# peterrum/deal-and-ceed-on-gpu

Hardware: AMD Instinct MI355X
Metric: BP5 DoFs/sec per CG iter (p=4, ~1e8 DoFs) + % HBM roofline at 1/2/4/8 GPUs (higher is better)
Workload: dtype f64

## Files before the change

deal-and-ceed-on-gpu_amd/csrc/bp5_device.hip:

```cpp
#include "bp5_device.hpp"


extern "C" int bp5_device_count(int *count)
{
  if (!count) return fail(BP5_ERR_INVALID, "null argument");
  int c = 0;
  hipError_t e = hipGetDeviceCount(&c);
  if (e != hipSuccess) { *count = 0; return fail(BP5_ERR_NO_DEVICE, hipGetErrorString(e)); }
  *count = c;
  return BP5_OK;
}
extern "C" int bp5_vec_alloc(size_t n, double **out)
{
  if (!out) return fail(BP5_ERR_INVALID, "null argument");
  HIP_TRY(hipMalloc((void **)out, std::max<size_t>(n, 1) * sizeof(double)));
  HIP_TRY(hipMemset(*out, 0, std::max<size_t>(n, 1) * sizeof(double)));
  HIP_TRY(hipStreamSynchronize(nullptr));
  return BP5_OK;
}
extern "C" int bp5_vec_free(double *v) { HIP_TRY(hipFree(v)); return BP5_OK; }
extern "C" int bp5_copy_h2d(void *dst, const void *src, size_t bytes) { HIP_TRY(hipMemcpy(dst, src, bytes, hipMemcpyHostToDevice)); return BP5_OK; }
extern "C" int bp5_copy_d2h(void *dst, const void *src, size_t bytes) { HIP_TRY(hipMemcpy(dst, src, bytes, hipMemcpyDeviceToHost)); return BP5_OK; }

static void tuning_from_environment(bp5_mf *mf);
// ... 701 lines not shown
    uint32_t *ra = lat.data() + g * BLOCK_LATTICE_WORDS, *rb = ra + BLOCK_LATTICE_WORDS;
    ra[55] = f.len << 16 | f.s_out;
    rb[56] = f.len << 16 | f.s_in;
    dp.h_carry_dof[g] = f.dof; dp.h_carry_len[g] = f.len;
    ++n_faces;
  }
  if (!n_faces) { dp.h_carry_dof.clear(); dp.h_carry_len.clear(); }
  return n_faces;
}

int build_carry_tables(bp5_mf *mf, bp5_mf::DevPlan *dp, const std::vector<uint32_t> &wb, uint32_t n_wg, bool two_parts, bp5_mf::DevPlan::CombineTables *out)
{
  std::vector<std::pair<uint32_t, uint32_t>> cut;
  for (int part = 0; part < (two_parts ? 2 : 1); ++part) {
    const uint32_t *w = wb.data() + (size_t)part * (n_wg + 1);
    for (uint32_t i = 0; i < n_wg; ++i)
      for (uint32_t g = w[i]; g + 1 < w[i + 1]; ++g)
        if (dp->h_carry_len[g]) cut.emplace_back(dp->h_carry_dof[g], dp->h_carry_len[g]);
  }
  std::sort(cut.begin(), cut.end());
  const std::vector<uint32_t> &st = dp->h_cr_start, &d0 = dp->h_cr_dof0, &so = dp->h_cr_soff, &sl = dp->h_cr_slots;
  const size_t nr = d0.size();
  std::vector<uint32_t> start, dof0, soff, slots;
  uint32_t ord = 0, owned = 0;
  size_t ci = 0;
  auto emit = [&](size_t r, uint32_t first, uint32_t count) {
    if (!count) return;
    const uint32_t base = d0[r] & 0x7fffffffu;
    start.push_back(ord);
    dof0.push_back(first | (d0[r] & 0x80000000u));
    soff.push_back((uint32_t)slots.size());
    for (uint32_t q = so[r]; q < so[r + 1]; ++q) slots.push_back(sl[q] + (first - base));
    ord += count;
    if (first < mf->n_owned) owned += std::min(count, mf->n_owned - first);
  };
  for (size_t r = 0; r < nr; ++r) {
    uint32_t first = d0[r] & 0x7fffffffu;
    const uint32_t end = first + (st[r + 1] - st[r]);
    while (ci < cut.size() && cut[ci].first + cut[ci].second <= first) ++ci;
    size_t c = ci;
    while (c < cut.size() && cut[c].first < end) {
      const uint32_t c0 = std::max(cut[c].first, first), c1 = std::min(cut[c].first + cut[c].second, end);
      emit(r, first, c0 - first);
      first = c1;
      ++c;
    }
    emit(r, first, end - first);
  }
  start.push_back(ord);
  soff.push_back((uint32_t)slots.size());
  BP5_TRY(upload_combine_tables(start, dof0, soff, slots, out));
  out->n_shared_owned = owned;
  return BP5_OK;
}

int get_plan_raw(bp5_mf *mf, int key, bp5_mf::DevPlan **dpo, int default_block)
{
  auto it = mf->plans.find(key);
  if (it == mf->plans.end()) {
    TeamPlanHost h;
    if (key < 0 && mf->n_local() >= (1ull << 30)) return fail(BP5_ERR_UNSUPPORTED, "block plan needs fewer than 2^30 local DoFs");
    if (key > 0) BP5_TRY(build_team_plan(mf->h_l2g.data(), mf->n_cells, mf->n3, mf->n_local(), key, h));
    else if (!mf->h_block_off.empty())
      BP5_TRY(build_team_plan(mf->h_l2g.data(), mf->n_cells, mf->n3, mf->n_local(), 0, h, mf->h_block_off.data(),
                              (uint32_t)mf->h_block_off.size() - 1, -key));
    else BP5_TRY(build_team_plan(mf->h_l2g.data(), mf->n_cells, mf->n3, mf->n_local(), default_block, h, nullptr, 0, -key));
    bp5_mf::DevPlan dp;
    BP5_TRY(upload(&dp.off, h.off.data(), h.off.size()));
    BP5_TRY(upload(&dp.dofs, h.dofs.data(), h.dofs.size()));
    std::vector<uint32_t> run_off, runs;
    if (key < 0) {
      std::vector<uint32_t> lat;
      std::vector<uint16_t> cpos;
      const bool lattice_enabled = mf->tune[BP5_TUNE_LATTICE_INDICES] != 0;
      dp.n_lattice_blocks = detect_lattice_blocks(mf->h_l2g.data(), mf->degree + 1, h.group_cell_off, h.off, h.dofs, lat, cpos);
      std::vector<CarryFace> faces;
      if (dp.n_lattice_blocks && dp.n_lattice_blocks == (uint32_t)(h.off.size() - 1)) faces = find_carry_faces(mf, mf->degree, h, lat);
      auto face_edge = [&](size_t g, uint32_t slot) {
        if (faces.empty()) return false;
        if (faces[g].len && (slot == faces[g].s_out || slot == faces[g].s_out + faces[g].len)) return true;
        return g > 0 && faces[g - 1].len && (slot == faces[g - 1].s_in || slot == faces[g - 1].s_in + faces[g - 1].len);
      };
      run_off.assign(h.off.size(), 0);
      for (size_t g = 0; g + 1 < h.off.size(); ++g) {
        uint32_t start = h.off[g];
        for (uint32_t i = h.off[g]; i < h.off[g + 1]; ++i) {
          const bool con = mf->h_constrained[h.dofs[i] & 0x7fffffffu];
          if (i == h.off[g] || h.dofs[i] != h.dofs[i - 1] + 1 || i - start == (1u << BLOCK_PACK_OFF_BITS) ||
              con != (bool)mf->h_constrained[h.dofs[i - 1] & 0x7fffffffu] || face_edge(g, i - h.off[g])) {
            start = i;
            runs.push_back(i - h.off[g]);
            runs.push_back(h.dofs[i] | (con ? BLOCK_DOF_CONSTRAINED : 0u));
          }
        }
        run_off[g + 1] = (uint32_t)(runs.size() / 2);
        dp.max_runs = std::max(dp.max_runs, run_off[g + 1] - run_off[g]);
      }
      const int n = mf->degree + 1, n2 = n * n;
      auto off = [&](int k, int ab) { return k < 2 * (n / 2) ? (k / 2) * (2 * n2) + 2 * ab + (k & 1) : (n / 2) * (2 * n2) + ab; };
      std::vector<uint16_t> pos2(h.pos.size()), packed(dp.max_runs <= (uint32_t)BLOCK_PACK_MAX_RUNS ? h.pos.size() : 0);
      std::vector<uint32_t> gidx(h.pos.size());
#pragma omp parallel
      {
        std::vector<uint16_t> run_of_slot;
#pragma omp for schedule(dynamic, 16)
        for (int64_t g = 0; g < (int64_t)h.group_cell_off.size() - 1; ++g) {
          const uint32_t nr = run_off[g + 1] - run_off[g], m = h.off[g + 1] - h.off[g];
          if (!packed.empty()) {
            run_of_slot.assign(m, 0);
            for (uint32_t r = 0; r < nr; ++r) {
              const uint32_t s0 = runs[2 * (run_off[g] + r)], s1 = r + 1 < nr ? runs[2 * (run_off[g] + r + 1)] : m;
              for (uint32_t sl = s0; sl < s1; ++sl) run_of_slot[sl] = (uint16_t)r;
            }
          }
          for (size_t c = h.group_cell_off[g]; c < h.group_cell_off[g + 1]; ++c)
            for (int k = 0; k < n; ++k)
              for (int ab = 0; ab < n2; ++ab) {
                const size_t from = c * mf->n3 + (size_t)k * n2 + ab, to = c * mf->n3 + off(k, ab);
                pos2[to] = h.pos[from];
                gidx[to] = mf->h_l2g[from];
                if (!packed.empty()) {
                  const uint32_t sl = h.pos[from], r = run_of_slot[sl];
                  packed[to] = (uint16_t)(r << BLOCK_PACK_OFF_BITS | (sl - runs[2 * (run_off[g] + r)]));
                }
              }
        }
      }
      BP5_TRY(upload(&dp.pos, pos2.data(), pos2.size()));
      BP5_TRY(upload(&dp.gidx, gidx.data(), gidx.size()));
      if (!packed.empty()) BP5_TRY(upload(&dp.packed, packed.data(), packed.size()));
      if (!packed.empty() && dp.n_lattice_blocks && lattice_enabled) {
        if (!faces.empty()) mark_carry_faces(h, faces, run_off, runs, lat, dp);
        BP5_TRY(upload(&dp.lattice, lat.data(), lat.size()));
        BP5_TRY(upload(&dp.cell_pos, cpos.data(), cpos.size()));
      } else
        dp.n_lattice_blocks = 0;
    } else
      BP5_TRY(upload(&dp.pos, h.pos.data(), h.pos.size()));
    BP5_TRY(upload(&dp.cell_round, h.cell_round.data(), h.cell_round.size()));
    BP5_TRY(upload(&dp.team_rounds, h.team_rounds.data(), h.team_rounds.size()));
    BP5_TRY(upload(&dp.sh_dof, h.sh_dof.data(), h.sh_dof.size()));
    BP5_TRY(upload(&dp.sh_off, h.sh_off.data(), h.sh_off.size()));
    BP5_TRY(upload(&dp.sh_slot, h.sh_slot.data(), h.sh_slot.size()));
    HIP_TRY(hipMalloc((void **)&dp.partial, std::max<size_t>(h.dofs.size(), 1) * sizeof(double)));
    HIP_TRY(hipMemsetAsync(dp.partial, 0, std::max<size_t>(h.dofs.size(), 1) * sizeof(double), mf->stream));
    BP5_TRY(upload(&dp.cell_off, h.group_cell_off.data(), h.group_cell_off.size()));
    if (key < 0) {
      BP5_TRY(upload(&dp.pass_cell, h.pass_cell.data(), h.pass_cell.size()));
      BP5_TRY(upload(&dp.pass_off, h.pass_off.data(), h.pass_off.size()));
      dp.h_cost.assign(h.pass_off.size(), 0.0);
      for (size_t g = 0; g + 1 < h.pass_off.size(); ++g) {
        const double passes = h.pass_off[g + 1] - h.pass_off[g], rounds = h.team_rounds[g], m = h.off[g + 1] - h.off[g];
        dp.h_cost[g + 1] = dp.h_cost[g] + passes * (1.0 + 0.18 * (rounds - 1.0)) + 1.5 * m / 4913.0 + 1.0;
      }
      runs.push_back(0); runs.push_back(0);
      BP5_TRY(upload(&dp.run_off, run_off.data(), run_off.size()));
      BP5_TRY(upload(&dp.runs, runs.data(), runs.size()));
    }
    dp.n_shared = (uint32_t)h.sh_dof.size();
    dp.n_shared_owned = (uint32_t)(std::lower_bound(h.sh_dof.begin(), h.sh_dof.end(), mf->n_owned) - h.sh_dof.begin());
    if (dp.n_shared) {
      std::vector<uint32_t> start, dof0, soff, slots, tile;
      const size_t ns = h.sh_dof.size();
      for (size_t i = 0; i < ns; ++i) {
        const uint32_t b = h.sh_off[i], e = h.sh_off[i + 1];
        bool cont = i > 0 && h.sh_dof[i] == h.sh_dof[i - 1] + 1 && (e - b) == (h.sh_off[i] - h.sh_off[i - 1]) &&
                    mf->h_constrained[h.sh_dof[i]] == mf->h_constrained[h.sh_dof[i - 1]];
        for (uint32_t q = 0; cont && q < e - b; ++q) cont = h.sh_slot[b + q] == h.sh_slot[h.sh_off[i - 1] + q] + 1;
        if (!cont) {
          start.push_back((uint32_t)i);
          dof0.push_back(h.sh_dof[i] | (mf->h_constrained[h.sh_dof[i]] ? 0x80000000u : 0u));
          soff.push_back((uint32_t)slots.size());
          slots.insert(slots.end(), h.sh_slot.begin() + b, h.sh_slot.begin() + e);
        }
      }
      start.push_back((uint32_t)ns);
      soff.push_back((uint32_t)slots.size());
      bp5_mf::DevPlan::CombineTables ct;
      BP5_TRY(upload_combine_tables(start, dof0, soff, slots, &ct));
      dp.cr_start = ct.start; dp.cr_dof0 = ct.dof0; dp.cr_soff = ct.soff; dp.cr_slots = ct.slots; dp.cr_tile = ct.tile;
      if (!dp.h_carry_len.empty()) { dp.h_cr_start = start; dp.h_cr_dof0 = dof0; dp.h_cr_soff = soff; dp.h_cr_slots = slots; }
    }
    dp.covers_all = h.covers_all;
    dp.n_groups = (uint32_t)h.group_cell_off.size() - 1;
    for (uint32_t g = 0; g < dp.n_groups; ++g) dp.max_list = std::max(dp.max_list, h.off[g + 1] - h.off[g]);
    it = mf->plans.emplace(key, dp).first;
  }
// ... 518 lines not shown
  for (hipEvent_t &e : mf->ev_halo) HIP_TRY(hipEventCreateWithFlags(&e, hipEventDisableTiming));
  int can = 0;
  if (hipDeviceGetAttribute(&can, hipDeviceAttributeCanUseStreamWaitValue, mf->device) != hipSuccess) can = 0;
  if (can && !mf->d_signal) {
    HIP_TRY(hipMalloc((void **)&mf->d_signal, 4 * sizeof(unsigned long long)));
    HIP_TRY(hipMemset(mf->d_signal, 0, 4 * sizeof(unsigned long long)));
    HIP_TRY(hipStreamSynchronize(nullptr));
    mf->signal_target = 0;
  }
  if (can) {
    mf->signal_target += 1;
    hipLaunchKernelGGL(wait_value_probe_producer, dim3(1), dim3(64), 0, mf->stream, mf->d_signal, mf->d_signal + 1, mf->d_signal + 2, 200000LL );
    KERNEL_CHECK();
    const bool waited = hipStreamWaitValue64(mf->comm_stream, mf->d_signal, mf->signal_target, hipStreamWaitValueGte, ~0ull) == hipSuccess;
    if (waited) { hipLaunchKernelGGL(wait_value_probe_consumer, dim3(1), dim3(64), 0, mf->comm_stream, mf->d_signal + 1); KERNEL_CHECK(); }
    else (void)hipGetLastError();
    HIP_TRY(hipStreamSynchronize(mf->stream));
    HIP_TRY(hipStreamSynchronize(mf->comm_stream));
    unsigned long long released_mid_kernel = 0;
    HIP_TRY(hipMemcpy(&released_mid_kernel, mf->d_signal + 2, sizeof(released_mid_kernel), hipMemcpyDeviceToHost));
    if (!waited || !released_mid_kernel) can = 0;
  }
  mf->wait_value_ok = can;
  mf->can_wait_value = can && mf->tune[BP5_TUNE_BOUNDARY_FIRST] != 0;
  return BP5_OK;
}
extern "C" int bp5_mf_wait_value_available(bp5_mf *mf, int *available)
{
  if (!mf || !available) return fail(BP5_ERR_INVALID, "null argument");
  HIP_TRY(hipSetDevice(mf->device));
  BP5_TRY(halo_streams(mf));
  *available = mf->wait_value_ok == 1;
  return BP5_OK;
}
static int env_int(const char *name, int fallback)
{
  const char *e = getenv(name);
  return (e && *e) ? atoi(e) : fallback;
}
static void tuning_from_environment(bp5_mf *mf)
{
  mf->tune[BP5_TUNE_LATTICE_INDICES] = env_int("BP5_LATTICE_INDICES", 1) != 0;
  mf->tune[BP5_TUNE_EARLY_GATHER] = env_int("BP5_EARLY_GATHER", 1) != 0;
  mf->tune[BP5_TUNE_COMBINE_SIGNAL] = env_int("BP5_COMBINE_SIGNAL", 0) == 1;
  { const char *e = getenv("BP5_BOUNDARY_FIRST"); mf->tune[BP5_TUNE_BOUNDARY_FIRST] = !(e && !strcmp(e, "launches")); }
  mf->tune[BP5_TUNE_FOLD_SMALL] = env_int("BP5_FOLD_SMALL", 1) != 0;
  { const int u = env_int("BP5_UPDATE_UNROLL", 1); mf->tune[BP5_TUNE_UPDATE_UNROLL] = (u == 2 || u == 4) ? u : 1; }
  mf->tune[BP5_TUNE_UPDATE_FLAT] = env_int("BP5_UPDATE_FLAT", 1) != 0;
  { const int v = env_int("BP5_UPDATE_NT", -1); mf->tune[BP5_TUNE_UPDATE_NT] = v < 0 ? -1 : v != 0; }
  { const int v = env_int("BP5_COMBINE_WG_PER_CU", 16); mf->tune[BP5_TUNE_COMBINE_WG_PER_CU] = (v >= 0 && v <= 32) ? v : 16; }
  mf->tune[BP5_TUNE_INTERIOR_STORES] = env_int("BP5_INTERIOR_STORES", 1) != 0;
  mf->tune[BP5_TUNE_GHOST_COMBINE_ON_COMM] = env_int("BP5_GHOST_COMBINE_ON_COMM", 0) != 0;
  mf->tune[BP5_TUNE_FACE_CARRY] = env_int("BP5_FACE_CARRY", 1) != 0;
}
extern "C" int bp5_mf_set_tuning(bp5_mf *mf, int knob, int value)
{
  if (!mf || knob < 0 || knob >= BP5_TUNE_COUNT) return fail(BP5_ERR_INVALID, "unknown tuning knob");
  switch (knob) {
    case BP5_TUNE_UPDATE_UNROLL:
      if (value != 1 && value != 2 && value != 4) return fail(BP5_ERR_INVALID, "BP5_TUNE_UPDATE_UNROLL: 1, 2 or 4");
      break;
    case BP5_TUNE_UPDATE_NT:
      if (value < -1 || value > 1) return fail(BP5_ERR_INVALID, "BP5_TUNE_UPDATE_NT: -1, 0 or 1");
      break;
    case BP5_TUNE_COMBINE_WG_PER_CU:
      if (value < 0 || value > 32) return fail(BP5_ERR_INVALID, "BP5_TUNE_COMBINE_WG_PER_CU: 0 ... 32");
      break;
    case BP5_TUNE_LATTICE_INDICES:
      if (value != 0 && value != 1) return fail(BP5_ERR_INVALID, "switch: 0 or 1");
      if (value != mf->tune[knob] && mf->plans.count(-block_cpt(mf))) return fail(BP5_ERR_INVALID, "BP5_TUNE_LATTICE_INDICES: the block plan of this handle is already built");
      break;
    default:
      if (value != 0 && value != 1) return fail(BP5_ERR_INVALID, "switch: 0 or 1");
  }
  mf->tune[knob] = value;
  if (knob == BP5_TUNE_BOUNDARY_FIRST && mf->wait_value_ok >= 0) mf->can_wait_value = mf->wait_value_ok == 1 && value != 0;
  return BP5_OK;
}
extern "C" int bp5_mf_get_tuning(const bp5_mf *mf, int knob, int *value)
{
  if (!mf || !value || knob < 0 || knob >= BP5_TUNE_COUNT) return fail(BP5_ERR_INVALID, "unknown tuning knob");
  *value = mf->tune[knob];
  return BP5_OK;
}
extern "C" int bp5_mf_set_overlap(bp5_mf *mf, int mode)
{
  if (!mf || mode < 0 || mode > 2) return fail(BP5_ERR_INVALID, "bad argument");
  mf->overlap = mode;
  return BP5_OK;
}
static bool overlap_wanted(const bp5_mf *mf) { return mf->overlap == 1 || (mf->overlap == 2 && mf->n_interior >= 1000000u); }
static int gather_exchange(bp5_mf *mf, double *v, bool on_comm_stream);
static int gather_start(bp5_mf *mf, double *v, bool on_comm_stream)
{
  HIP_TRY(hipSetDevice(mf->device));
  BP5_TRY(halo_streams(mf));
  const uint32_t ns = mf->send_off.back();
  if (ns) {
    hipLaunchKernelGGL(pack_kernel, dim3((ns + 255) / 256), dim3(256), 0, mf->stream, mf->d_send_idx, ns, v, mf->d_sendbuf);
    KERNEL_CHECK();
  }
  return gather_exchange(mf, v, on_comm_stream);
}
extern "C" int bp5_halo_gather_start(bp5_mf *mf, double *v)
{
  if (!mf || !v) return fail(BP5_ERR_INVALID, "null argument");
  if (mf->neighbors.empty()) return BP5_OK;
  if (!mf->comm) return fail(BP5_ERR_INVALID, "halo exchange needs bp5_mf_set_comm");
  return gather_start(mf, v, overlap_wanted(mf));
}
static int gather_exchange(bp5_mf *mf, double *v, bool on_comm_stream)
{
  mf->overlap_now = on_comm_stream;
  hipStream_t cs = mf->overlap_now ? mf->comm_stream : mf->stream;
  if (mf->overlap_now) {
    HIP_TRY(hipEventRecord(mf->ev_halo[0], mf->stream));
// ... 368 lines not shown
extern "C" int bp5_event_elapsed_ms(bp5_event *a, bp5_event *b, double *ms)
{
  if (!a || !b || !ms) return fail(BP5_ERR_INVALID, "null argument");
  HIP_TRY(hipEventSynchronize(b->ev));
  float f = 0.f;
  HIP_TRY(hipEventElapsedTime(&f, a->ev, b->ev));
  *ms = f;
  return BP5_OK;
}
extern "C" int bp5_event_destroy(bp5_event *e)
{
  if (!e) return BP5_OK;
  hipEventDestroy(e->ev);
  delete e;
  return BP5_OK;
}

static int ensure_ws(bp5_mf *mf)
{
  if (mf->ws_g) return BP5_OK;
  const size_t stagger = 0;
  const size_t nb = (std::max<size_t>(mf->n_local(), 2) * sizeof(double) + 4095) / 4096 * 4096;
  char *base = nullptr;
  HIP_TRY(hipMalloc((void **)&base, 3 * nb + 2 * stagger + 4096));
  HIP_TRY(hipMemsetAsync(base, 0, 3 * nb + 2 * stagger + 4096, mf->stream));
  mf->ws_base = base;
  mf->ws_g = (double *)base;
  mf->ws_d = (double *)(base + nb + stagger);
  mf->ws_h = (double *)(base + 2 * nb + 2 * stagger);
  return BP5_OK;
}

struct ApplyProfile {
  bp5_mf *mf;
  bool on;
  int used = 0;
  static constexpr int MAX_PROFILED = 512;
  int mark(int k)
  {
    if (!on) return BP5_OK;
    if (used >= 4 * MAX_PROFILED) { on = false; return BP5_OK; }
    while ((size_t)used + 4 > mf->ev_pool.size()) { hipEvent_t e; HIP_TRY(hipEventCreate(&e)); mf->ev_pool.push_back(e); }
    HIP_TRY(hipEventRecord(mf->ev_pool[used + k], mf->stream));
    return BP5_OK;
  }
};

struct SolveState {
  ApplyProfile prof;
  int exchange = EXCHANGE_NONE;
  bool two_parts = false;
  bool gather_in_flight = false;
  bool dst_prezeroed = false, copies_dirichlet = false;
  bool phase_on = false;
  int phase_it = 0;
  uint8_t phase_recorded[bp5_mf::PhaseProfile::MAX_ITERS] = {};
};

static int phase_mark(bp5_mf *mf, SolveState &ss, int k)
{
  if (!ss.phase_on || ss.phase_it >= bp5_mf::PhaseProfile::MAX_ITERS) return BP5_OK;
  HIP_TRY(hipEventRecord(mf->phase.ev[(size_t)ss.phase_it * bp5_mf::PhaseProfile::MARKS + k], mf->stream));
  ss.phase_recorded[ss.phase_it] |= (uint8_t)(1u << k);
  return BP5_OK;
}

static int fused_unsplit(bp5_mf *mf, SolveState &ss, ApplyCall &call, const double *coef, const double *src, double *dst)
{
  ApplyProfile &prof = ss.prof;
  if (prof.on) call.mark_event = mf->ev_pool[prof.used + 2];
  BP5_TRY(launch_apply(mf, call, coef, src, dst));
  if (!call.mark_recorded) BP5_TRY(prof.mark(2));
  BP5_TRY(prof.mark(3));
  if (prof.on) prof.used += 4;
  BP5_TRY(phase_mark(mf, ss, 3));
  BP5_TRY(halo_streams(mf));
  BP5_TRY(scatter_exchange(mf, dst, false));
  return scatter_add_finish(mf, dst, call.fuse);
}
static int fused_ghost_rows_first(bp5_mf *mf, SolveState &ss, ApplyCall &call, const double *coef, const double *src, double *dst)
{
  ApplyProfile &prof = ss.prof;
  bp5_mf::DevPlan *dp = nullptr;
  BP5_TRY(get_plan_raw(mf, -block_cpt(mf), &dp));
  BP5_TRY(halo_streams(mf));
  call.combine_later = true;
  BP5_TRY(launch_apply(mf, call, coef, src, dst));
  BP5_TRY(prof.mark(2));
  const bool combine_signal = mf->tune[BP5_TUNE_COMBINE_SIGNAL] != 0;
  const bool one_combine = combine_signal && mf->can_wait_value == 1 && mf->n_ghost && mf->d_signal && dp->n_shared > dp->n_shared_owned && dp->cr_tile && !call.csr_combine;
  if (one_combine) {
    BP5_TRY(launch_combine(mf, call, dp, dst, true, COMBINE_GHOST_THEN_OWNED));
    HIP_TRY(hipStreamWaitValue64(mf->comm_stream, mf->d_signal, mf->signal_target, hipStreamWaitValueGte, ~0ull));
    BP5_TRY(scatter_exchange(mf, dst, true, true));
  } else if (mf->tune[BP5_TUNE_GHOST_COMBINE_ON_COMM] && mf->n_ghost) {
    HIP_TRY(hipEventRecord(mf->ev_halo[2], mf->stream));
    HIP_TRY(hipStreamWaitEvent(mf->comm_stream, mf->ev_halo[2], 0));
    BP5_TRY(launch_combine(mf, call, dp, dst, true, COMBINE_GHOST, true));
    BP5_TRY(scatter_exchange(mf, dst, true, true));
    BP5_TRY(launch_combine(mf, call, dp, dst, true, COMBINE_OWNED));
  } else {
    if (mf->n_ghost) BP5_TRY(launch_combine(mf, call, dp, dst, true, COMBINE_GHOST));
    BP5_TRY(scatter_exchange(mf, dst, true));
    BP5_TRY(launch_combine(mf, call, dp, dst, true, mf->n_ghost ? COMBINE_OWNED : COMBINE_ALL));
  }
  BP5_TRY(prof.mark(3));
// ... 41 lines not shown
  if (ss.gather_in_flight) { ss.gather_in_flight = false; BP5_TRY(bp5_halo_gather_finish(mf, src)); }
  else {
    BP5_TRY(gather_start(mf, src, false));
    BP5_TRY(bp5_halo_gather_finish(mf, src));
  }
  BP5_TRY(phase_mark(mf, ss, 2));
  BP5_TRY(ss.prof.mark(0));
  BP5_TRY(ss.prof.mark(1));
  FuseState fuse;
  fuse.p = src; fuse.r = fuse_r;
  ApplyCall call;
  call.c0 = 0; call.c1 = mf->n_cells; call.overwrite = true;
  call.fuse = &fuse;
  call.exchange = ss.exchange;
  call.two_parts = ss.two_parts;
  if (ss.exchange == EXCHANGE_BOUNDARY_FIRST) BP5_TRY(fused_boundary_first(mf, ss, call, coef, src, dst));
  else if (ss.exchange == EXCHANGE_GHOST_ROWS_FIRST) BP5_TRY(fused_ghost_rows_first(mf, ss, call, coef, src, dst));
  else BP5_TRY(fused_unsplit(mf, ss, call, coef, src, dst));
  *n_cols = fuse.n_cols;
  if (!fuse.ghosts_zeroed) BP5_TRY(bp5_halo_zero_ghosts(mf, src));
  return BP5_OK;
}

static int solver_vmult(bp5_mf *mf, SolveState &ss, const double *coef, double *src, double *dst, bool zero, const double *fuse_r = nullptr,
                        uint32_t *n_cols = nullptr)
{
  ApplyProfile &prof = ss.prof;
  const bool dist = mf->has_neighbors();
  const bool fusing = n_cols != nullptr;
  if (dist && fusing) return fused_vmult_distributed(mf, ss, coef, src, dst, fuse_r, n_cols);
  ApplyCall call;
  call.c0 = 0; call.c1 = mf->n_cells;
  if (dist) {
    BP5_TRY(prof.mark(0));
    BP5_TRY(prof.mark(1));
    if (prof.on) call.mark_event = mf->ev_pool[prof.used + 2];
    BP5_TRY(apply_overlapped(mf, call, coef, src, dst, zero));
    if (!call.mark_recorded) BP5_TRY(prof.mark(2));
    BP5_TRY(prof.mark(3));
    if (prof.on) prof.used += 4;
    BP5_TRY(bp5_halo_zero_ghosts(mf, src));
    return bp5_copy_constrained(mf, src, dst);
  }
  const bool owner_scatter = variant_overwrites(mf, effective_variant(mf, 0, mf->n_cells));
  BP5_TRY(prof.mark(0));
  if (zero && !owner_scatter) {
    if (!ss.dst_prezeroed) HIP_TRY(hipMemsetAsync(dst, 0, mf->n_local() * sizeof(double), mf->stream));
    zero = false;
    call.dst_known_zero = true;
  }
  BP5_TRY(prof.mark(1));
  if (prof.on) call.mark_event = mf->ev_pool[prof.used + 2];
  FuseState fuse;
  if (fusing) { fuse.p = src; fuse.r = fuse_r; call.fuse = &fuse; }
  call.overwrite = zero;
  BP5_TRY(launch_apply(mf, call, coef, src, dst));
  if (fusing) *n_cols = fuse.n_cols;
  if (!call.mark_recorded) BP5_TRY(prof.mark(2));
  BP5_TRY(prof.mark(3));
  if (prof.on) prof.used += 4;
  if (fusing) return BP5_OK;
  if (ss.copies_dirichlet) return BP5_OK;
  return bp5_copy_constrained(mf, src, dst);
}

static int poll_state(bp5_mf *mf)
{
  HIP_TRY(hipMemcpyAsync(mf->h_st, mf->d_st, ST_COUNT * sizeof(int), hipMemcpyDeviceToHost, mf->stream));
  HIP_TRY(hipMemcpyAsync(mf->h_sc, mf->d_sc, SC_COUNT * sizeof(double), hipMemcpyDeviceToHost, mf->stream));
  HIP_TRY(hipStreamSynchronize(mf->stream));
  return BP5_OK;
}

static int solve_begin(bp5_mf *mf, const bp5_cg_params *prm, const ApplyProfile &prof)
{
  hipStream_t s = mf->stream;
  if (prof.on) {
    const size_t want = 4 * (size_t)std::min(prm->max_iter, ApplyProfile::MAX_PROFILED);
    while (mf->ev_pool.size() < want) { hipEvent_t e; HIP_TRY(hipEventCreate(&e)); mf->ev_pool.push_back(e); }
  }
  mf->h_sc[SC_TOL] = prm->abs_tol;
  HIP_TRY(hipMemcpyAsync(mf->d_sc + SC_TOL, mf->h_sc + SC_TOL, sizeof(double), hipMemcpyHostToDevice, s));
  mf->h_st[ST_MAXIT] = prm->max_iter;
  HIP_TRY(hipMemcpyAsync(mf->d_st + ST_MAXIT, mf->h_st + ST_MAXIT, sizeof(int), hipMemcpyHostToDevice, s));
  HIP_TRY(hipStreamSynchronize(s));
  HIP_TRY(hipEventRecord(mf->ev_solve[0], s));
  return BP5_OK;
}
static int solve_finish(bp5_mf *mf, const ApplyProfile &prof, bool fused_dots, int exchange_schedule, bool own_operator, bp5_cg_result *res)
{
  HIP_TRY(hipEventRecord(mf->ev_solve[1], mf->stream));
  BP5_TRY(poll_state(mf));
  float ms = 0.f;
  HIP_TRY(hipEventElapsedTime(&ms, mf->ev_solve[0], mf->ev_solve[1]));
  memset(res, 0, sizeof(*res));
  res->iterations = mf->h_st[ST_ITER];
  res->residual = mf->h_sc[SC_RES];
  res->initial_residual = mf->h_sc[SC_RES0];
  res->solve_ms = ms;
  res->apply_launches = prof.used / 4;
  res->dot_products_fused = fused_dots ? 1 : 0;
  res->exchange_schedule = exchange_schedule;
  if (prof.on && prof.used) {
    double tot = 0.0, tot_op = 0.0;
    for (int k = 0; k < prof.used; k += 4) {
      float t = 0.f;
      HIP_TRY(hipEventElapsedTime(&t, mf->ev_pool[k + 1], mf->ev_pool[k + 2]));
      tot += t;
      HIP_TRY(hipEventElapsedTime(&t, mf->ev_pool[k], mf->ev_pool[k + 3]));
      tot_op += t;
    }
    res->apply_ms_avg = tot / (prof.used / 4);
    res->operator_ms_avg = tot_op / (prof.used / 4);
  }
  if (own_operator) strncpy(res->apply_kernel, mf->last_apply_kernel, sizeof(res->apply_kernel) - 1);
  if (mf->h_st[ST_BREAKDOWN]) return fail(BP5_ERR_BREAKDOWN, "CG breakdown: p.Ap is zero or NaN");
  return BP5_OK;
}

static int user_vmult(ApplyProfile &prof, bp5_vmult_fn user, void *user_ctx, double *src, double *dst)
{
  BP5_TRY(prof.mark(0));
  BP5_TRY(prof.mark(1));
  const int st = user(user_ctx, dst, src);
  if (st != BP5_OK) return fail(st, "the operator's vmult callback reported a failure");
  BP5_TRY(prof.mark(2));
  BP5_TRY(prof.mark(3));
  if (prof.on) prof.used += 4;
  return BP5_OK;
}

struct OperatorPlan {
  bool dist = false;
  bool fused_dots = false;
  bool fold_small = false;
  bool prezero = false;
  int schedule = 0;
};
static int plan_operator(bp5_mf *mf, bool own_operator, bool fusable, SolveState &ss, OperatorPlan &op)
{
  op.dist = mf->has_neighbors();
  bool split = false, split_possible = false, late = false;
  if (own_operator && mf->cg_fusion && !mf->f32_metric()  && fusable && mf->geometry_mode == BP5_GEOM_MERGED6 &&
      is_default_block(mf, effective_variant(mf, 0, mf->n_cells))) {
    bp5_mf::DevPlan *dp = nullptr;
    BP5_TRY(get_plan_raw(mf, -block_cpt(mf), &dp));
    op.fused_dots = dp->packed && dp->covers_all && (dp->n_shared == 0 || dp->cr_tile);
    if (op.fused_dots && op.dist) {
      uint32_t b0_, b1_;
      split_possible = !mf->h_block_off.empty() && (mf->n_interior == 0 || mf->n_interior == mf->n_cells || block_aligned(mf, 0, mf->n_interior, &b0_, &b1_));
      split = split_possible && mf->overlap == 1;
      if (mf->overlap == 1 && !split) op.fused_dots = false;
      late = op.fused_dots && mf->overlap == 2 && (dp->n_shared == 0 || dp->cr_tile);
    }
  }
  ss.exchange = split ? EXCHANGE_BOUNDARY_FIRST : late ? EXCHANGE_GHOST_ROWS_FIRST : EXCHANGE_NONE;
  ss.two_parts = op.fused_dots && op.dist && split_possible;
  const bool fold_enabled = mf->tune[BP5_TUNE_FOLD_SMALL] != 0;
  op.fold_small = fold_enabled && !op.fused_dots && own_operator && !op.dist;
  op.prezero = op.fold_small && mf->n_ghost == 0 && !variant_overwrites(mf, effective_variant(mf, 0, mf->n_cells));
  ss.dst_prezeroed = op.prezero;
  ss.copies_dirichlet = op.fold_small;
  op.schedule = !op.dist ? 0 : split ? 2 : late ? 4 : op.fused_dots ? 1 : overlap_wanted(mf) ? 3 : 1;
  return BP5_OK;
}

struct PlainCG {
  int n_components = 1;
  size_t ld = 0;
  double *g = nullptr, *d = nullptr, *h = nullptr;
  const double *coef = nullptr;
  bp5_vmult_fn user = nullptr;
  void *user_ctx = nullptr;
  bool block = false, exchange = false;
  const double *diag = nullptr;
  bp5_vmult_fn precond = nullptr;
  void *precond_ctx = nullptr;
  double *z = nullptr;
  bool allreduce = true;
  double *history = nullptr;
  int history_cap = 0;
};
static int cg_solve_plain(bp5_mf *mf, const PlainCG &cg, const double *b, double *x, const bp5_cg_params *prm, bp5_cg_result *res)
{
  hipStream_t s = mf->stream;
  const size_t n = mf->n_owned, ld = cg.ld;
  const int nc = cg.n_components;
  double *g = cg.g, *d = cg.d, *h = cg.h, *z = cg.z;
  const double *diag = cg.diag;
  const int cols = PARTIAL_STRIDE / nc;
  const dim3 grid1(std::min(stream_grid(n, 1), cols), nc), grid2(std::min(stream_grid(n, 2), cols), nc), block(VB);
  const dim3 gridd = cg.block ? grid2 : dim3(stream_grid_flat(mf, n, 2));
  const int nblk1 = (int)grid1.x * nc, nblk2 = (int)grid2.x * nc;
  const int *no_flag = nullptr;
  SolveState ss{ApplyProfile{mf, prm->profile != 0 && !cg.precond}};
  ApplyProfile &prof = ss.prof;
  BP5_TRY(solve_begin(mf, prm, prof));
  OperatorPlan op;
  if (!cg.block && !cg.precond) BP5_TRY(plan_operator(mf, !cg.user, true, ss, op));
  else op.schedule = cg.user || !mf->has_neighbors() ? 0 : overlap_wanted(mf) ? 3 : 1;
  auto apply_A = [&](uint32_t *n_cols) -> int {
    if (cg.user) return user_vmult(prof, cg.user, cg.user_ctx, d, h);
    if (!cg.block) return solver_vmult(mf, ss, cg.coef, d, h, true, nullptr, op.fused_dots ? n_cols : nullptr);
    BP5_TRY(prof.mark(0));
    BP5_TRY(components_zero(mf, nc, ld, h));
    BP5_TRY(prof.mark(1));
    if (cg.exchange) BP5_TRY(components_apply_exchanged(mf, cg.coef, nc, ld, d, h, false));
// ... 53 lines not shown
    } else {
      hipLaunchKernelGGL(cg_update_kernel<true>, grid2, block, 0, s, x, g, d, h, diag, n, ld, mf->d_sc, mf->d_st, mf->d_partials, op.prezero);
      hipLaunchKernelGGL(finalize_kernel<2>, dim3(2), block, 0, s, mf->d_partials, nblk2, mf->d_sc + SC_GG, mf->d_st);
    }
    if (cg.allreduce) { KERNEL_CHECK(); BP5_TRY(bp5_comm_allreduce_sum(mf, mf->d_sc + SC_GG, 2)); }
    hipLaunchKernelGGL(cg_control_kernel, dim3(1), dim3(1), 0, s, mf->d_sc, mf->d_st);
    if (cg.history) hipLaunchKernelGGL(cg_record_kernel, dim3(1), dim3(1), 0, s, mf->d_sc, mf->d_st, cg.history, cg.history_cap);
    if (cg.precond) hipLaunchKernelGGL((cg_direction_kernel<true, false>), gridd, block, 0, s, d, z, diag, n, ld, mf->d_sc, mf->d_st);
    else hipLaunchKernelGGL((cg_direction_kernel<false, false>), gridd, block, 0, s, d, g, diag, n, ld, mf->d_sc, mf->d_st);
    KERNEL_CHECK();
    if (check > 0 && it % check == 0 && it < prm->max_iter) {
      BP5_TRY(poll_state(mf));
      if (mf->h_st[ST_DONE]) break;
    } else if (lagged_look && it < prm->max_iter) {
      const int slot = it % (DONE_LAG + 1);
      HIP_TRY(hipMemcpyAsync(mf->h_done + slot, mf->d_st + ST_DONE, sizeof(int), hipMemcpyDeviceToHost, s));
      HIP_TRY(hipEventRecord(mf->ev_done[slot], s));
      if (it > DONE_LAG) {
        const int seen = (it - DONE_LAG) % (DONE_LAG + 1);
        HIP_TRY(hipEventSynchronize(mf->ev_done[seen]));
        if (mf->h_done[seen]) break;
      }
    }
  }
  return solve_finish(mf, prof, op.fused_dots, op.schedule, !cg.user, res);
}

static int cg_solve_merged(bp5_mf *mf, const double *coef, bp5_vmult_fn user, void *user_ctx, const double *diag, const double *b, double *x,
                           const bp5_cg_params *prm, bp5_cg_result *res)
{
  const size_t n = mf->n_owned;
  const int grid2 = stream_grid(n, 2), grid1 = stream_grid(n, 1);
  hipStream_t s = mf->stream;
  double *g = mf->ws_g, *d = mf->ws_d, *h = mf->ws_h;
  SolveState ss{ApplyProfile{mf, prm->profile != 0}};
  ss.phase_on = prm->profile == 2;
  if (ss.phase_on) {
    const size_t want = (size_t)bp5_mf::PhaseProfile::MAX_ITERS * bp5_mf::PhaseProfile::MARKS;
    while (mf->phase.ev.size() < want) { hipEvent_t e; HIP_TRY(hipEventCreate(&e)); mf->phase.ev.push_back(e); }
  }
  BP5_TRY(solve_begin(mf, prm, ss.prof));
  OperatorPlan op;
  BP5_TRY(plan_operator(mf, !user, !diag, ss, op));
  const bool fused = op.fused_dots, dist_solve = op.dist, fold_small = op.fold_small, prezero = op.prezero;
  auto vmult = [&](double *src, double *dst, const double *fuse_r, uint32_t *n_cols) -> int {
    if (!user) return solver_vmult(mf, ss, coef, src, dst, true, fuse_r, n_cols);
    return user_vmult(ss.prof, user, user_ctx, src, dst);
  };
  const int check = prm->check_every;
  hipLaunchKernelGGL(cgm_init_kernel, dim3(grid1), dim3(VB), 0, s, b, x, g, d, h, diag, n, mf->d_partials, !(fused && !dist_solve));
  hipLaunchKernelGGL(finalize_kernel<2>, dim3(2), dim3(VB), 0, s, mf->d_partials, grid1, mf->d_sc + SC_GG, (const int *)nullptr);
  KERNEL_CHECK();
  BP5_TRY(bp5_comm_allreduce_sum(mf, mf->d_sc + SC_GG, 2));
  hipLaunchKernelGGL(cgm_init_control_kernel, dim3(1), dim3(1), 0, s, mf->d_sc, mf->d_st);
  KERNEL_CHECK();
  const int unroll = mf->tune[BP5_TUNE_UPDATE_UNROLL];
  const int gridu = stream_grid_flat(mf, n, 2 * unroll);
  const bool streaming = mf->tune[BP5_TUNE_UPDATE_NT] != 0;
  auto launch_update = [&](int mode) {
#define BP5_UPD(M, U, ZV, NT) hipLaunchKernelGGL((cgm_update_kernel<M, U, ZV, NT>), dim3(gridu), dim3(VB), 0, s, d, g, h, x, diag, n, mf->d_sc, mf->d_st)
#define BP5_UPD_U(M, ZV, NT) do { if (unroll == 1) BP5_UPD(M, 1, ZV, NT); else if (unroll == 2) BP5_UPD(M, 2, ZV, NT); else BP5_UPD(M, 4, ZV, NT); } while (0)
    if (mode == 0) { BP5_UPD_U(0, false, false); return; }
    if (prezero) { if (mode == 1) BP5_UPD_U(1, true, false); else BP5_UPD_U(2, true, false); return; }
    if (streaming) { if (mode == 1) BP5_UPD_U(1, false, true); else BP5_UPD_U(2, false, true); return; }
    if (mode == 1) BP5_UPD_U(1, false, false); else BP5_UPD_U(2, false, false);
#undef BP5_UPD_U
#undef BP5_UPD
  };
  const bool early_gather_enabled = mf->tune[BP5_TUNE_EARLY_GATHER] != 0;
  const bool early_gather = fused && dist_solve && early_gather_enabled;
  auto gather_under_update = [&](int mode) -> int {
    BP5_TRY(halo_streams(mf));
    const uint32_t ns = mf->send_off.back();
    if (ns) {
      const dim3 gr((ns + 255) / 256), bl(256);
      if (mode == 0) hipLaunchKernelGGL(cgm_pack_updated_kernel<0>, gr, bl, 0, s, mf->d_send_idx, ns, d, g, h, diag, mf->d_sc, mf->d_st, mf->d_sendbuf);
      else hipLaunchKernelGGL(cgm_pack_updated_kernel<1>, gr, bl, 0, s, mf->d_send_idx, ns, d, g, h, diag, mf->d_sc, mf->d_st, mf->d_sendbuf);
      KERNEL_CHECK();
    }
    return gather_exchange(mf, d, true);
  };
  int it = 1;
  for (; it <= prm->max_iter; ++it) {
    const int mode = it == 1 ? 0 : it % 2 == 0 ? 1 : 2;
    BP5_TRY(phase_mark(mf, ss, 0));
    if (early_gather) { BP5_TRY(gather_under_update(mode)); ss.gather_in_flight = true; }
    if (mode != 0) launch_update(mode);
    KERNEL_CHECK();
    BP5_TRY(phase_mark(mf, ss, 1));
    const bool one_launch = fused && !mf->comm;
    if (fused) {
      uint32_t n_cols = 0;
      BP5_TRY(vmult(d, h, g, &n_cols));
      BP5_TRY(phase_mark(mf, ss, 4));
      if (one_launch) hipLaunchKernelGGL(cgm_finalize4_kernel<true>, dim3(1), dim3(FIN4_THREADS), 0, s, mf->d_partials, (int)n_cols, mf->d_sc, mf->d_st);
      else hipLaunchKernelGGL(cgm_finalize4_kernel<false>, dim3(1), dim3(FIN4_THREADS), 0, s, mf->d_partials, (int)n_cols, mf->d_sc, mf->d_st);
    } else {
      BP5_TRY(vmult(d, h, nullptr, nullptr));
      BP5_TRY(phase_mark(mf, ss, 4));
      hipLaunchKernelGGL(cgm_dots_kernel, dim3(grid2), dim3(VB), 0, s, d, g, h, diag, n, mf->d_st, mf->d_partials,
                         fold_small ? (const uint32_t *)mf->d_constrained_bits : (const uint32_t *)nullptr);
      hipLaunchKernelGGL(finalize_kernel<7>, dim3(7), dim3(VB), 0, s, mf->d_partials, grid2, mf->d_sc + SC_R0, mf->d_st);
    }
    KERNEL_CHECK();
    BP5_TRY(phase_mark(mf, ss, 5));
    if (!one_launch) {
      BP5_TRY(bp5_comm_allreduce_sum(mf, mf->d_sc + SC_R0, 7));
      BP5_TRY(phase_mark(mf, ss, 6));
      hipLaunchKernelGGL(cgm_control_kernel, dim3(1), dim3(1), 0, s, mf->d_sc, mf->d_st);
      KERNEL_CHECK();
    } else
      BP5_TRY(phase_mark(mf, ss, 6));
    BP5_TRY(phase_mark(mf, ss, 7));
    if (ss.phase_on) ++ss.phase_it;
    if (check > 0 && it % check == 0 && it < prm->max_iter) {
      BP5_TRY(poll_state(mf));
      if (mf->h_st[ST_DONE]) break;
    }
  }
  if (prm->max_iter > 0) {
    launch_update(1);
    hipLaunchKernelGGL(cgm_control_kernel, dim3(1), dim3(1), 0, s, mf->d_sc, mf->d_st);
    KERNEL_CHECK();
  }
  const int status = solve_finish(mf, ss.prof, fused, op.schedule, !user, res);
  if (!ss.phase_on || (status != BP5_OK && status != BP5_ERR_BREAKDOWN)) return status;
  using PP = bp5_mf::PhaseProfile;
  const int n_it = std::min(ss.phase_it, (int)PP::MAX_ITERS);
  int counted = 0;
  for (int i = n_it > 1 ? 1 : 0; i < n_it; ++i) {
    const uint8_t rec = ss.phase_recorded[i];
    const uint8_t need = (1u << 0) | (1u << 1) | (1u << 4) | (1u << 5) | (1u << 6) | (1u << 7);
    if ((rec & need) != need) continue;
    auto ms = [&](int a, int b, double &out) -> int {
      float t = 0.f;
      HIP_TRY(hipEventElapsedTime(&t, mf->phase.ev[(size_t)i * PP::MARKS + a], mf->phase.ev[(size_t)i * PP::MARKS + b]));
      out += t;
      return BP5_OK;
    };
    const bool g = rec & (1u << 2), x = rec & (1u << 3);
    BP5_TRY(ms(0, 1, res->phase_ms[BP5_PHASE_UPDATE]));
    if (g) BP5_TRY(ms(1, 2, res->phase_ms[BP5_PHASE_GATHER_WAIT]));
    BP5_TRY(ms(g ? 2 : 1, x ? 3 : 4, res->phase_ms[BP5_PHASE_OPERATOR]));
    if (x) BP5_TRY(ms(3, 4, res->phase_ms[BP5_PHASE_EXCHANGE]));
    BP5_TRY(ms(4, 5, res->phase_ms[BP5_PHASE_REDUCE]));
    BP5_TRY(ms(5, 6, res->phase_ms[BP5_PHASE_ALLREDUCE]));
    BP5_TRY(ms(6, 7, res->phase_ms[BP5_PHASE_CONTROL]));
    BP5_TRY(ms(0, 7, res->phase_ms[BP5_PHASE_ITERATION]));
    ++counted;
  }
  if (counted) for (double &v : res->phase_ms) v /= counted;
  return status;
}

static int cg_solve_impl(bp5_mf *mf, const double *coef, bp5_vmult_fn user, void *user_ctx, const double *diag, const double *b, double *x,
                         const bp5_cg_params *prm, bp5_cg_result *res, double *history = nullptr, int history_cap = 0)
{
  if (!mf || (!user && !coef && mf->geometry_mode != BP5_GEOM_AFFINE) || !b || !x || !prm || !res) return fail(BP5_ERR_INVALID, "null argument");
  if (prm->max_iter < 0) return fail(BP5_ERR_INVALID, "max_iter < 0");
  if (prm->variant != BP5_CG_PLAIN && prm->variant != BP5_CG_MERGED) return fail(BP5_ERR_INVALID, "unknown CG variant");
  if (!aligned16(b) || !aligned16(x) || (diag && !aligned16(diag))) return fail(BP5_ERR_INVALID, "vectors must be 16-byte aligned");
  HIP_TRY(hipSetDevice(mf->device));
  BP5_TRY(ensure_ws(mf));
  if (prm->variant == BP5_CG_MERGED) return cg_solve_merged(mf, coef, user, user_ctx, diag, b, x, prm, res);
  PlainCG cg;
  cg.g = mf->ws_g; cg.d = mf->ws_d; cg.h = mf->ws_h;
  cg.coef = coef; cg.user = user; cg.user_ctx = user_ctx;
  cg.diag = diag;
  cg.history = history; cg.history_cap = history_cap;
  return cg_solve_plain(mf, cg, b, x, prm, res);
}

extern "C" int bp5_cg_solve(bp5_mf *mf, const double *coef, const double *diag, const double *b, double *x, const bp5_cg_params *prm,
                            bp5_cg_result *res)
// ... 693 lines not shown
```

deal-and-ceed-on-gpu_amd/csrc/bp5_device.hpp:

```cpp
#pragma once
#include "bp5_internal.hpp"
#include "bp5_kernels.hpp"

#include <hip/hip_runtime.h>
#include <rccl/rccl.h>

#include <algorithm>
#include <cmath>
#include <cstdio>
#include <cstdlib>
#include <cstring>
#include <map>
#include <memory>
#include <tuple>
#include <vector>

using namespace bp5;

#define HIP_TRY(expr)                                                                                              \
  do {                                                                                                             \
    hipError_t e_ = (expr);                                                                                        \
    if (e_ != hipSuccess)                                                                                          \
      return fail(e_ == hipErrorNoDevice || e_ == hipErrorInvalidDevice ? BP5_ERR_NO_DEVICE : BP5_ERR_HIP,         \
                  std::string(#expr) + ": " + hipGetErrorString(e_));                                              \
// ... 13 lines not shown
struct bp5_comm {
  ncclComm_t comm = nullptr;
  int rank = 0, n_ranks = 1;
};
struct bp5_event {
  hipEvent_t ev = nullptr;
};

constexpr size_t STREAMING_MAX_DOFS = 24000000;
struct bp5_mf {
  int degree = 0, quadrature = 0, coefficient = 0, n = 0, n3 = 0, device = 0;
  int nq = 0, nq3 = 0;
  bool overint() const { return quadrature == BP5_QUAD_GAUSS_OVER; }
  uint32_t n_cells = 0, n_interior = 0, n_owned = 0, n_ghost = 0, n_constrained = 0;
  int apply_variant = 0, n_cus = 0, geometry_mode = 0, march_max_steps = 32;
  int operator_kind = 0;
  mutable int coef_planes_committed = 0;
  static int planes_of(int op) { return op == BP5_OP_HELMHOLTZ ? 7 : op == BP5_OP_MASS ? 1 : 6; }
  int n_planes() const { return planes_of(operator_kind); }
  int metric_precision = BP5_METRIC_F64;
  bool f32_metric() const { return metric_precision == BP5_METRIC_F32; }
  int block_max_wg = 0;
  int streaming = -1;
  int auto_team = -1;
  int auto_block = -1;
  double *d_scalar_plane = nullptr, *d_gcell = nullptr;
  hipStream_t stream = nullptr;
  bool own_stream = false;
  Tables tab, tab_gauss;
  uint32_t *d_l2g = nullptr, *d_constrained = nullptr, *d_send_idx = nullptr;
  uint32_t *d_constrained_bits = nullptr;
  double *d_coords = nullptr, *d_tab = nullptr, *d_tab_gauss = nullptr;
  uint32_t *d_l2g_padded = nullptr, *d_constraint_mask = nullptr;
  uint64_t coef_plane_stride = 0, coef_cell_stride = 0;
  bool has_hanging = false;
  uint32_t *d_hang_mask = nullptr;
  double *d_hang_I = nullptr;
  double *d_inv_jac = nullptr, *d_JxW = nullptr, *d_qpoints = nullptr;
  uint32_t pad = 0;
  std::vector<int> neighbors;
  std::vector<uint32_t> send_off, recv_off;
  double *d_sendbuf = nullptr, *d_recvbuf = nullptr;
  uint8_t *d_send_dirichlet = nullptr;
  bp5_comm *comm = nullptr;
  hipStream_t comm_stream = nullptr;
  hipEvent_t ev_halo[4] = {nullptr, nullptr, nullptr, nullptr};
  int overlap = 2;
  bool overlap_now = false;
  bool cg_fusion = true;
  unsigned long long *d_signal = nullptr;
  uint64_t signal_target = 0;
  int wait_value_ok = -1;
  int can_wait_value = -1;
  int tune[BP5_TUNE_COUNT] = {1, 1, 0, 1, 1, 1, 1, -1, 16, 1, 0, 1};
  bool cell_interiors_first = false;
  double *d_partials = nullptr, *d_sc = nullptr, *d_scalar = nullptr;
  int *d_st = nullptr;
  double *ws_g = nullptr, *ws_d = nullptr, *ws_h = nullptr, *d_evec = nullptr;
  char *ws_base = nullptr;
  double *ws_z = nullptr;
  double *wsc_base = nullptr;
  size_t wsc_cap = 0;
  double *hc_base = nullptr;
  size_t hc_cap = 0;
  uint32_t *d_hc_off = nullptr;
  int *h_done = nullptr;
  hipEvent_t ev_done[3] = {nullptr, nullptr, nullptr};
  unsigned long long *d_stamps = nullptr;
  double *h_sc = nullptr;
  int *h_st = nullptr;
  std::vector<hipEvent_t> ev_pool;
  hipEvent_t ev_solve[2] = {nullptr, nullptr};
  char last_apply_kernel[96] = "";
  struct PhaseProfile {
    static constexpr int MARKS = 8, MAX_ITERS = 64;
    std::vector<hipEvent_t> ev;
  } phase;
  std::vector<uint32_t> h_l2g;
  struct DevPlan {
    uint32_t *off = nullptr, *dofs = nullptr, *sh_dof = nullptr, *sh_off = nullptr, *sh_slot = nullptr;
    uint16_t *pos = nullptr;
    uint8_t *cell_round = nullptr, *team_rounds = nullptr;
    double *partial = nullptr;
    uint32_t *cell_off = nullptr, *pass_cell = nullptr, *pass_off = nullptr, *run_off = nullptr, *runs = nullptr, *gidx = nullptr;
    uint16_t *packed = nullptr;
    uint32_t *lattice = nullptr;
    uint16_t *cell_pos = nullptr;
    uint32_t n_lattice_blocks = 0;
    std::vector<double> h_cost;
    std::map<std::tuple<uint32_t, uint32_t, uint32_t, uint32_t>, uint32_t *> *wg_blocks = nullptr;
    uint32_t *cr_start = nullptr, *cr_dof0 = nullptr, *cr_soff = nullptr, *cr_slots = nullptr, *cr_tile = nullptr;
    struct CombineTables { uint32_t *start = nullptr, *dof0 = nullptr, *soff = nullptr, *slots = nullptr, *tile = nullptr; uint32_t n_shared = 0, n_shared_owned = 0; };
    std::vector<uint32_t> h_cr_start, h_cr_dof0, h_cr_soff, h_cr_slots;
    std::vector<uint32_t> h_carry_dof, h_carry_len;
    std::map<std::tuple<uint32_t, uint32_t, uint32_t, uint32_t>, CombineTables> *cr_carry = nullptr;
    const CombineTables *cr_last_launch = nullptr;
    uint32_t n_shared = 0, n_groups = 0, max_list = 0, max_runs = 0;
    uint32_t n_shared_owned = 0;
    bool covers_all = false;
  };
  std::vector<bool> h_constrained;
  std::vector<uint32_t> h_block_off;
  struct DevMarch { uint32_t *team_off = nullptr, *entries = nullptr; uint32_t n_teams = 0; };
  std::map<int, DevMarch> march_plans;
  std::map<int, DevPlan> plans;
  size_t n_local() const { return (size_t)n_owned + n_ghost; }
  bool has_neighbors() const { return comm && !neighbors.empty(); }
};

struct FuseState {
  const double *p = nullptr, *r = nullptr;
  uint32_t n_cols = 0;
  bool ghosts_zeroed = false;
};
enum VariantFamily { VARIANT_PENCIL, VARIANT_TEAM, VARIANT_MARCH, VARIANT_BLOCK, VARIANT_BLOCK_SIBLING, VARIANT_HANGING_PENCIL, VARIANT_OTHER };
struct VariantInfo {
  VariantFamily family;
  bool atomic_scatter;
  bool shared_by_atomics;
  bool csr_combine;
  bool overwrites;
};
constexpr VariantInfo decode_variant(int v)
{
  const int b = v % 100;
  const VariantFamily f = b <= 6 ? VARIANT_PENCIL : b >= 10 && b <= 14 ? VARIANT_TEAM : b == 56 ? VARIANT_BLOCK : b >= 48 && b <= 63 ? VARIANT_BLOCK_SIBLING
                        : b >= 70 && b <= 72 ? VARIANT_MARCH : b == 90 ? VARIANT_HANGING_PENCIL : VARIANT_OTHER;
  return {f, v >= 100, b == 54 || b == 55, b == 48, v < 100 && (f == VARIANT_TEAM || f == VARIANT_BLOCK || f == VARIANT_BLOCK_SIBLING)};
}

enum { EXCHANGE_NONE = 0, EXCHANGE_BOUNDARY_FIRST = 1, EXCHANGE_GHOST_ROWS_FIRST = 2 };
struct ApplyCall {
  uint32_t c0 = 0, c1 = 0;
  bool overwrite = false;
  bool dst_known_zero = false;
  int variant = 0;
  bool keep_variant = false;
  bool atomic_scatter = false, shared_by_atomics = false, csr_combine = false;
  void set_variant(int v)
  {
    const VariantInfo d = decode_variant(v);
    variant = v; atomic_scatter = d.atomic_scatter; shared_by_atomics = d.shared_by_atomics; csr_combine = d.csr_combine;
  }
  uint32_t b0 = 0, b1 = 0;
  bool combine_later = false;
  bool two_parts = false, signal = false;
  int exchange = EXCHANGE_NONE;
  FuseState *fuse = nullptr;
  hipEvent_t mark_event = nullptr;
  bool mark_recorded = false;
  const bp5_mf::DevPlan::CombineTables *combine_tables = nullptr;
};

#ifndef BP5_LPC_P2
#define BP5_LPC_P2 9
#endif
#ifndef BP5_LPC_P5
#define BP5_LPC_P5 36
#endif
#ifndef BP5_LPC_P8
#define BP5_LPC_P8 81
#endif
constexpr int block_lpc(int degree) { return degree == 1 ? 4 : degree == 2 ? BP5_LPC_P2 : degree == 3 ? 16 : degree == 4 ? 32 : degree == 5 ? BP5_LPC_P5 : degree == 6 || degree == 7 ? 64 : degree == 8 ? BP5_LPC_P8 : 0; }
inline int block_cpt(const bp5_mf *mf) { return block_lpc(mf->degree) ? 256 / block_lpc(mf->degree) : 8; }

template <typename T>
// ... 215 lines not shown
      std::vector<uint32_t> wb((two_parts ? 2 : 1) * (size_t)(n_wg + 1));
      if (!two_parts) {
        const double c0 = pc[B0], total = pc[B1] - c0;
        for (uint32_t w = 0; w <= n_wg; ++w)
          wb[w] = (uint32_t)(std::lower_bound(pc.begin() + B0, pc.begin() + B1 + 1, c0 + total * w / n_wg - 1e-9) - pc.begin());
        wb[0] = B0; wb[n_wg] = B1;
      } else {
        uint32_t *wa = wb.data(), *wi = wb.data() + n_wg + 1;
        const double ca = pc[Bs], ta = pc[B1] - ca, ci = pc[B0], ti = pc[Bs] - ci;
        for (uint32_t w = 0; w <= n_wg; ++w) {
          wa[w] = (uint32_t)(std::lower_bound(pc.begin() + Bs, pc.begin() + B1 + 1, ca + ta * w / n_wg - 1e-9) - pc.begin());
          if (w == 0) wa[w] = Bs;
          if (w == n_wg) wa[w] = B1;
          const double want = (ta + ti) * w / n_wg - (pc[wa[w]] - ca);
          wi[w] = (uint32_t)(std::lower_bound(pc.begin() + B0, pc.begin() + Bs + 1, ci + std::max(want, 0.0) - 1e-9) - pc.begin());
          if (w > 0) wi[w] = std::max(wi[w], wi[w - 1]);
        }
        wi[0] = B0; wi[n_wg] = Bs;
      }
      return wb;
    };
    if (itw == dp->wg_blocks->end()) {
      const std::vector<uint32_t> wb = make_ranges();
      uint32_t *dev = nullptr;
      BP5_TRY(upload(&dev, wb.data(), wb.size()));
      itw = dp->wg_blocks->emplace(key, dev).first;
    }
    bp.wg_block = itw->second;
    call.combine_tables = nullptr;
    if constexpr ((ABL & BLK_CARRY) != 0) {
      if (mf->tune[BP5_TUNE_FACE_CARRY] && !sub_range && !atomic_shared && dp->cr_tile && !call.csr_combine && !dp->h_carry_len.empty()) {
        if (!dp->cr_carry) dp->cr_carry = new std::map<std::tuple<uint32_t, uint32_t, uint32_t, uint32_t>, bp5_mf::DevPlan::CombineTables>;
        auto itc = dp->cr_carry->find(key);
        if (itc == dp->cr_carry->end()) {
          bp5_mf::DevPlan::CombineTables ct;
          BP5_TRY(build_carry_tables(mf, dp, make_ranges(), n_wg, two_parts, &ct));
          itc = dp->cr_carry->emplace(key, ct).first;
        }
        if (itc->second.n_shared < dp->n_shared) {
          call.combine_tables = &itc->second;
          bp.carry = 1u;
        }
      }
    }
    dp->cr_last_launch = call.combine_tables;
    bp.n_parts = two_parts ? 2u : 1u;
    bp.signal = nullptr;
    if (call.signal) {
      if (!two_parts || !mf->d_signal) return fail(BP5_ERR_INVALID, "boundary-first signal: the launch has no separate ghost-touching part");
      bp.signal = mf->d_signal;
    }
  }
  bp.cg_r = call.fuse ? call.fuse->r : nullptr; bp.dot_partials = mf->d_partials; bp.n_owned = mf->n_owned; bp.cg_state = mf->d_st;
  bp.stamps = nullptr;
  if (ABL & BLK_STAMPS) {
    if (!mf->d_stamps) HIP_TRY(hipMalloc((void **)&mf->d_stamps, 4096 * 16 * sizeof(unsigned long long)));
    HIP_TRY(hipMemsetAsync(mf->d_stamps, 0, 4096 * 16 * sizeof(unsigned long long), mf->stream));
    bp.stamps = mf->d_stamps;
  }
  ApplyArgs a = apply_args(mf, (ABL & BLK_AFFINE) != 0, coef, src, dst);
  a.cell_begin = 0; a.cell_end = mf->n_cells; a.n_teams = dp->n_groups; a.teams_per_xcd = 0;
  if ((ABL & BLK_HANG) && !mf->has_hanging) return fail(BP5_ERR_INVALID, "the hanging-node build needs constraint masks");
  ShapeArg<n> sh;
  fill_shape(sh, mf);
  const bool set = overwrite && dp->covers_all;
  if (overwrite && !set) BP5_TRY(zero_dst(mf, dst));
  if (bp.signal && atomic_shared) return fail(BP5_ERR_INVALID, "boundary-first signal: owner-store launches only");
  const dim3 grid(n_wg), block(256);
  snprintf(mf->last_apply_kernel, sizeof(mf->last_apply_kernel), "apply_block_kernel<%d,%s,%d,%d,%d>", P, COLL ? "true" : "false", LPC,
           atomic_shared ? (set ? SC_OWNER_SET_ATOMIC : SC_OWNER_ADD_ATOMIC) : (set ? SC_OWNER_SET : SC_OWNER_ADD), ABL);
  if constexpr ((ABL & BLK_FUSE) != 0) {
    if (!set || atomic_shared || (sub_range && !call.combine_later) || (call.combine_later && call.exchange == EXCHANGE_NONE) || !call.fuse)
      return fail(BP5_ERR_INVALID, "fused dot products need overwrite launches that cover the whole range");
    if (call.fuse->n_cols + n_wg > (uint32_t)PARTIAL_STRIDE / 2) return fail(BP5_ERR_UNSUPPORTED, "too many workgroups for the partial-sum rows");
    bp.dot_col0 = call.fuse->n_cols;
    call.fuse->n_cols += n_wg;
  }
  if constexpr ((ABL & BLK_FUSE) == 0) if (atomic_shared) {
    if (set && dp->n_shared) {
      hipLaunchKernelGGL(zero_indexed_kernel, dim3((dp->n_shared + 255) / 256), dim3(256), 0, mf->stream, dp->sh_dof, dp->n_shared, dst);
      KERNEL_CHECK();
    }
    if (set) {
      auto kern = apply_block_kernel<P, COLL, LPC, SC_OWNER_SET_ATOMIC, ABL>;
      HIP_TRY(hipFuncSetAttribute((const void *)kern, hipFuncAttributeMaxDynamicSharedMemorySize, (int)lds));
      hipLaunchKernelGGL(kern, grid, block, lds, mf->stream, a, bp, sh);
    } else {
      auto kern = apply_block_kernel<P, COLL, LPC, SC_OWNER_ADD_ATOMIC, ABL>;
      HIP_TRY(hipFuncSetAttribute((const void *)kern, hipFuncAttributeMaxDynamicSharedMemorySize, (int)lds));
      hipLaunchKernelGGL(kern, grid, block, lds, mf->stream, a, bp, sh);
    }
    KERNEL_CHECK();
    return BP5_OK;
  }
  if (set) {
    auto kern = apply_block_kernel<P, COLL, LPC, SC_OWNER_SET, ABL>;
    HIP_TRY(hipFuncSetAttribute((const void *)kern, hipFuncAttributeMaxDynamicSharedMemorySize, (int)lds));
    hipLaunchKernelGGL(kern, grid, block, lds, mf->stream, a, bp, sh);
  } else if constexpr ((ABL & BLK_FUSE) == 0) {
    auto kern = apply_block_kernel<P, COLL, LPC, SC_OWNER_ADD, ABL>;
    HIP_TRY(hipFuncSetAttribute((const void *)kern, hipFuncAttributeMaxDynamicSharedMemorySize, (int)lds));
    hipLaunchKernelGGL(kern, grid, block, lds, mf->stream, a, bp, sh);
  }
  KERNEL_CHECK();
  if (bp.signal) mf->signal_target += n_wg;
  if (ABL & BLK_STAMPS) {
// ... 42 lines not shown
    KERNEL_CHECK();
    return launch_combine(mf, call, dp, dst, set);
  }
  KERNEL_CHECK();
  return BP5_OK;
}
#define BP5_UNPAREN(...) __VA_ARGS__
#define LAUNCH_COLL(FN, P, TARGS, ...)                                                                             \
  (coll ? FN<P, true, BP5_UNPAREN TARGS>(mf, call, __VA_ARGS__) : FN<P, false, BP5_UNPAREN TARGS>(mf, call, __VA_ARGS__))
#define TEAM_CASE(P, V, TW, LPC, PF) BP5_CASE(P, V) return LAUNCH_COLL(launch_team_t, P, (TW, LPC, PF), coef, src, dst, c0, c1, overwrite)

template <int P, bool COLL, int TW, int LPC, bool PF, int ABL = 0>
inline int launch_march_t(bp5_mf *mf, ApplyCall &, const double *coef, const double *src, double *dst, bool overwrite)
{
  constexpr int n = P + 1;
  constexpr int CPT = 64 * TW / LPC;
  using L = LdsLayout<n, LPC>;
  auto it = mf->march_plans.find(CPT);
  if (it == mf->march_plans.end()) {
    MarchPlanHost h;
    BP5_TRY(build_march_plan(mf->h_l2g.data(), mf->n_cells, n, CPT, mf->march_max_steps, h));
    bp5_mf::DevMarch dm;
    BP5_TRY(upload(&dm.team_off, h.team_off.data(), h.team_off.size()));
    BP5_TRY(upload(&dm.entries, h.entries.data(), h.entries.size()));
    dm.n_teams = (uint32_t)h.team_off.size() - 1;
    it = mf->march_plans.emplace(CPT, dm).first;
  }
  MarchPlan mp{};
  mp.team_off = it->second.team_off; mp.entries = it->second.entries; mp.n_teams = it->second.n_teams;
  mp.teams_per_xcd = (mp.n_teams + 7) / 8;
  if (overwrite) BP5_TRY(zero_dst(mf, dst));
  ApplyArgs a = apply_args(mf, (ABL & BLK_AFFINE) != 0, coef, src, dst);
  a.cell_begin = 0; a.cell_end = mf->n_cells; a.n_teams = mp.n_teams; a.teams_per_xcd = mp.teams_per_xcd;
  ShapeArg<n> sh;
  fill_shape(sh, mf);
  const size_t lds = (size_t)CPT * L::CS * sizeof(double);
  snprintf(mf->last_apply_kernel, sizeof(mf->last_apply_kernel), "apply_march_kernel<%d,%s,%d,%d,%s,%d>", P, COLL ? "true" : "false", TW, LPC, PF ? "true" : "false", ABL);
  hipLaunchKernelGGL((apply_march_kernel<P, COLL, TW, LPC, PF, ABL>), dim3(mp.teams_per_xcd * 8), dim3(64 * TW), lds, mf->stream, a, mp, sh);
  KERNEL_CHECK();
  return BP5_OK;
}

template <int M, bool GAUSS_ONLY = false> struct Bld {};
template <typename... B> struct BuildList {};
template <int DEG>
struct DefaultBlockBuilds {
  static constexpr int D = BLK_DEFAULT, F = BLK_FUSE;
  using list = BuildList<Bld<D | BLK_LATT>, Bld<D | F | BLK_LATT>, Bld<D>, Bld<D | F>, Bld<D | BLK_F32M | BLK_LATT>, Bld<D | BLK_F32M>, Bld<D | BLK_HELM>,
                         Bld<D | F | BLK_HELM>, Bld<D | BLK_MASS>, Bld<D | F | BLK_MASS>, Bld<D | BLK_HANG>, Bld<D | F | BLK_HANG>>;
};
template <>
struct DefaultBlockBuilds<4> {
  static constexpr int D = BLK_DEFAULT, F = BLK_FUSE, LATC = BLK_LATT | BLK_CARRY;
  using list = BuildList<Bld<D | LATC | BLK_NTM, true>, Bld<D | F | LATC | BLK_NTM, true>, Bld<D | LATC>, Bld<D | F | LATC>, Bld<D>, Bld<D | F>,
#ifdef BP5_TIMING_BUILDS
                         Bld<D | BLK_LATT | BLK_NTM | BLK_ROLL, true>, Bld<D | F | BLK_LATT | BLK_NTM | BLK_ROLL, true>, Bld<D | BLK_LATT | BLK_ROLL, true>,
                         Bld<D | F | BLK_LATT | BLK_ROLL, true>,
#endif
                         Bld<D | BLK_F32M | LATC>, Bld<D | BLK_F32M>, Bld<D | BLK_HELM>, Bld<D | F | BLK_HELM>, Bld<D | BLK_MASS>, Bld<D | F | BLK_MASS>, Bld<D | BLK_HANG | BLK_NTM, true>,
                         Bld<D | F | BLK_HANG | BLK_NTM, true>, Bld<D | BLK_HANG>, Bld<D | F | BLK_HANG>, Bld<D | BLK_AFFINE>,
                         Bld<BLK_SINGLE | BLK_SEQ | BLK_RUNS>, Bld<BLK_SINGLE | BLK_SEQ>>;
};
constexpr int BLK_OPTIONAL = BLK_LATT | BLK_CARRY | BLK_NTM;
constexpr bool build_serves(int m, bool gauss_only, int want, bool coll)
{
  return (m & ~BLK_OPTIONAL) == (want & ~BLK_OPTIONAL) && (m & BLK_OPTIONAL & ~want) == 0 && !(gauss_only && coll);
}
template <int DEG, int M, bool GAUSS_ONLY>
inline bool launch_if_serves(Bld<M, GAUSS_ONLY>, int want, int *status, bp5_mf *mf, ApplyCall &call, const double *coef, const double *src, double *dst)
{
  const bool coll = mf->quadrature == BP5_QUAD_GLL;
  if (!build_serves(M, GAUSS_ONLY, want, coll)) return false;
  if constexpr (GAUSS_ONLY) *status = launch_block_t<DEG, false, block_lpc(DEG), M>(mf, call, coef, src, dst, call.overwrite);
  else *status = LAUNCH_COLL(launch_block_t, DEG, (block_lpc(DEG), M), coef, src, dst, call.overwrite);
  return true;
}
template <int DEG, typename... B>
inline bool launch_first_that_serves(BuildList<B...>, int want, int *status, bp5_mf *mf, ApplyCall &call, const double *coef, const double *src, double *dst)
{
  return (launch_if_serves<DEG>(B{}, want, status, mf, call, coef, src, dst) || ...);
}
template <int DEG>
inline int launch_block_default(bp5_mf *mf, ApplyCall &call, const double *coef, const double *src, double *dst)
{
  static_assert(block_lpc(DEG) != 0, "no block-kernel shape for this degree");
  const int variant = call.variant % 100;
  if (!block_aligned(mf, call.c0, call.c1, &call.b0, &call.b1)) return fail(BP5_ERR_INVALID, "variant 56 needs a cell range aligned with the cell blocks");
  bp5_mf::DevPlan *dp = nullptr;
  BP5_TRY(get_plan_raw(mf, -(256 / block_lpc(DEG)), &dp));
  const int cls =
      mf->f32_metric() ? BLK_F32M : mf->operator_kind == BP5_OP_HELMHOLTZ ? BLK_HELM : mf->operator_kind == BP5_OP_MASS ? BLK_MASS : mf->has_hanging ? BLK_HANG : mf->geometry_mode == BP5_GEOM_AFFINE ? BLK_AFFINE : 0;
  int want;
  if (dp->packed && variant != 49) {
    want = BLK_DEFAULT | cls | (call.fuse ? BLK_FUSE : 0);
    if (dp->lattice && dp->n_lattice_blocks == dp->n_groups && variant != 48) want |= BLK_LATT | BLK_CARRY;
    if (streaming_accesses(mf)) want |= BLK_NTM;
  } else {
    if (DEG != 4 || cls != 0) return fail(BP5_ERR_UNSUPPORTED, "variant " + std::to_string(variant) + " needs packed indices (<= 128 runs per cell block)");
    if (call.fuse) return fail(BP5_ERR_INVALID, "fused dot products need the packed block kernel");
    want = dp->max_runs <= (uint32_t)BLOCK_MAX_RUNS ? BLK_SINGLE | BLK_SEQ | BLK_RUNS : BLK_SINGLE | BLK_SEQ;
  }
#ifndef BP5_TIMING_BUILDS
  if (variant == 63) return fail(BP5_ERR_INVALID, "variant 63 lives in libbp5_timing.so");
#else
  if (variant == 63) {
    if (!(want & BLK_LATT) || mf->quadrature == BP5_QUAD_GLL) return fail(BP5_ERR_UNSUPPORTED, "variant 63 (rolling metric prefetch) needs lattice blocks and Gauss quadrature");
    want = (want & ~BLK_CARRY) | BLK_ROLL;
  }
#endif
  int status = BP5_OK;
  if (!launch_first_that_serves<DEG>(typename DefaultBlockBuilds<DEG>::list{}, want, &status, mf, call, cls == BLK_AFFINE ? mf->d_scalar_plane : coef, src, dst))
    return fail(BP5_ERR_UNSUPPORTED, "the block kernel has no build for this operator, plan and solver request");
  return status;
}

#define APPLY_CASE(P, V, TW, LPC, TPB, PF) BP5_CASE(P, V) return LAUNCH_COLL(launch_apply_t, P, (TW, LPC, TPB, PF), coef, src, dst, c0, c1, overwrite)

template <int P>
inline int launch_affine(bp5_mf *mf, ApplyCall &call, const double *src, double *dst, uint32_t c0, uint32_t c1, bool overwrite)
{
  const bool coll = mf->quadrature == BP5_QUAD_GLL;
  return LAUNCH_COLL(launch_apply_t, P, (4, (P + 1) * (P + 1), 1, true, BLK_AFFINE), mf->d_scalar_plane, src, dst, c0, c1, overwrite);
}

#define BP5_CASE(P, V) if constexpr (DEG == (P)) if (variant == (V))
#define LAUNCH_DEFAULT_PENCIL(ABL, COEF) LAUNCH_COLL(launch_apply_t, DEG, (DP::TW, DP::LPC, DP::TPB, DP::PF, ABL), COEF, src, dst, c0, c1, overwrite)
template <int DEG>
int apply_degree_impl(bp5_mf *mf, ApplyCall &call, const double *coef, const double *src, double *dst)
{
  using DP = DefaultPencil<DEG>;
  const uint32_t c0 = call.c0, c1 = call.c1;
  const bool overwrite = call.overwrite;
  const bool coll = mf->quadrature == BP5_QUAD_GLL;
  const bool affine = mf->geometry_mode == BP5_GEOM_AFFINE;
  if (c1 <= c0) return overwrite ? zero_dst(mf, dst) : BP5_OK;
  if (mf->overint()) return overint_apply(mf, call, coef, src, dst);
  if (mf->f32_metric()) {
    if (mf->operator_kind != BP5_OP_POISSON || mf->has_hanging || affine)
      return fail(BP5_ERR_UNSUPPORTED, "FP32 metric planes: Poisson operator on a conforming mesh with the six-plane geometry only");
    if (call.fuse) return fail(BP5_ERR_UNSUPPORTED, "FP32 metric planes: no fused dot products");
    if (call.variant == 56) return launch_block_default<DEG>(mf, call, coef, src, dst);
    if (call.variant != 0) return fail(BP5_ERR_UNSUPPORTED, "FP32 metric planes run apply variants 0 (pencil kernel) and 56 (block kernel)");
    return LAUNCH_DEFAULT_PENCIL(BLK_F32M, coef);
  }
  if (mf->operator_kind == BP5_OP_HELMHOLTZ) {
    if (mf->has_hanging || affine) return fail(BP5_ERR_UNSUPPORTED, "the Helmholtz operator needs a conforming mesh and the six-plane geometry");
    if (call.variant == 56) return launch_block_default<DEG>(mf, call, coef, src, dst);
#ifdef BP5_TIMING_BUILDS
    if constexpr (DEG == 3) if (call.variant == 91 || call.variant == 93 || call.variant == 95) {
// ... 217 lines not shown
```

deal-and-ceed-on-gpu_amd/csrc/bp5_kernels.hpp:

```cpp
#pragma once
#include <hip/hip_runtime.h>
#include <stdint.h>
#include <type_traits>

namespace bp5 {

template <int n>
struct ShapeArg {
  double N[n * n];
  double D[n * n];
};

enum : int {
  BLK_AFFINE = 1024, BLK_SINGLE = 2048, BLK_STAMPS = 4096, BLK_SEQ = 8192, BLK_RUNS = 16384, BLK_NTM = 32768, BLK_PACK = 262144,
  BLK_STAGE = 524288, BLK_FUSE = 1048576, BLK_HANG = 2097152, BLK_LDSADD = 4194304, BLK_HELM = 8388608, BLK_LATT = 16777216,
  BLK_ROLL = 67108864, BLK_CARRY = 268435456,
  BLK_F32M = 536870912,
  BLK_MASS = 1073741824,
  BLK_DEFAULT = BLK_SINGLE | BLK_SEQ | BLK_RUNS | BLK_PACK
};
enum : int {
  PEN_INTERIOR_STORES = 32,
  PEN_NT_LOADS = 256,
  PEN_FULL_OCCUPANCY = 512
};
enum : int { TEAM_DIRECT_GATHER = 32 };

template <int n>
__host__ __device__ constexpr int coef_off(int qi, int ab)
{
  return (qi < 2 * (n / 2)) ? (qi / 2) * (2 * n * n) + 2 * ab + (qi & 1) : (n / 2) * (2 * n * n) + ab;
}
typedef double bp5_d2u __attribute__((ext_vector_type(2), aligned(8)));
template <int n, bool NT = false>
__device__ __forceinline__ void load_pencil(const double *base, int ab, double (&S)[n])
{
#pragma unroll
  for (int m = 0; m < n / 2; ++m) {
    const bp5_d2u *q = reinterpret_cast<const bp5_d2u *>(base + m * (2 * n * n) + 2 * ab);
    const bp5_d2u v = NT ? __builtin_nontemporal_load(q) : *q;
    S[2 * m] = v.x;
    S[2 * m + 1] = v.y;
  }
  if constexpr (n & 1) S[n - 1] = NT ? __builtin_nontemporal_load(base + (n / 2) * (2 * n * n) + ab) : base[(n / 2) * (2 * n * n) + ab];
}

typedef float bp5_f2u __attribute__((ext_vector_type(2), aligned(4)));
template <int n, bool NT = false>
__device__ __forceinline__ void load_pencil(const float *base, int ab, float (&S)[n])
{
#pragma unroll
  for (int m = 0; m < n / 2; ++m) {
    const bp5_f2u *q = reinterpret_cast<const bp5_f2u *>(base + m * (2 * n * n) + 2 * ab);
    const bp5_f2u v = NT ? __builtin_nontemporal_load(q) : *q;
    S[2 * m] = v.x;
    S[2 * m + 1] = v.y;
  }
  if constexpr (n & 1) S[n - 1] = NT ? __builtin_nontemporal_load(base + (n / 2) * (2 * n * n) + ab) : base[(n / 2) * (2 * n * n) + ab];
}
template <int ABL> using metric_t = typename std::conditional<(ABL & BLK_F32M) != 0, float, double>::type;

template <int n, bool NT = false>
__device__ __forceinline__ void load_pencil_pair(const double *base, int ab, int m, double &s0, double &s1)
{
  const bp5_d2u *q = reinterpret_cast<const bp5_d2u *>(base + m * (2 * n * n) + 2 * ab);
  const bp5_d2u v = NT ? __builtin_nontemporal_load(q) : *q;
  s0 = v.x;
// ... 940 lines not shown
    for (int k = 0; k < n; ++k) acc += y[k];
    if (acc == 1.2345e300) a.dst[gidx[0] & 0x7fffffffu] = acc + my_round + n_rounds;
    return;
  }
  __syncthreads();
#pragma unroll
  for (int r = 0; r < MAXU; ++r) {
    const int i = t + r * TEAM;
    if (i < m) lds[i] = 0.0;
  }
  __syncthreads();
  for (int rd = 0; rd < n_rounds; ++rd) {
    if (active && my_round == rd) {
#pragma unroll
      for (int k = 0; k < n; ++k) lds[ps[k]] += y[k];
    }
    __syncthreads();
  }
#pragma unroll
  for (int r = 0; r < MAXU; ++r) {
    const int i = t + r * TEAM;
    if (i < m) {
      const double v = lds[i];
      const uint32_t g = gidx[r];
      if constexpr (SCATTER == SC_ATOMIC) {
        atomic_add_f64(a.dst + (g & 0x7fffffffu), v);
      } else {
        if (g & 0x80000000u) {
          if constexpr (SCATTER == SC_OWNER_SET) a.dst[g & 0x7fffffffu] = v;
          else a.dst[g & 0x7fffffffu] += v;
        } else
          tp.partial[o0 + i] = v;
      }
    }
  }
#undef TL
}


template <int n, typename T>
__device__ __forceinline__ void load_pencil_idx(const T *base, int ab, T (&v)[n])
{
  typedef T pair_t __attribute__((ext_vector_type(2), aligned(sizeof(T))));
#pragma unroll
  for (int m = 0; m < n / 2; ++m) {
    const pair_t q = *reinterpret_cast<const pair_t *>(base + m * (2 * n * n) + 2 * ab);
    v[2 * m] = q.x;
    v[2 * m + 1] = q.y;
  }
  if constexpr (n & 1) v[n - 1] = base[(n / 2) * (2 * n * n) + ab];
}

__device__ __forceinline__ void lds_drain() { asm volatile("s_waitcnt lgkmcnt(0)" ::: "memory"); }

struct ComponentArgs {
  uint32_t n_components;
  uint64_t ld;
};
#ifndef BP5_COMPONENTS_PREFETCH_MAX_DEGREE
#define BP5_COMPONENTS_PREFETCH_MAX_DEGREE 6
#endif
constexpr bool components_gather_prefetch(int degree) { return degree <= BP5_COMPONENTS_PREFETCH_MAX_DEGREE; }
#ifndef BP5_COMPONENTS_P8_WAVES
#define BP5_COMPONENTS_P8_WAVES 2
#endif
constexpr int components_waves_per_simd(int degree, bool coll) { return degree == 8 && !coll ? BP5_COMPONENTS_P8_WAVES : 1; }
template <int P, bool COLL, int TW, int LPC, int TPB>
__global__ void __launch_bounds__(64 * TW * TPB, components_waves_per_simd(P, COLL)) apply_pencil_components_kernel(ApplyArgs a, ComponentArgs ca, ShapeArg<P + 1> sh)
{
  constexpr int n = P + 1, n2 = n * n, n3 = n2 * n;
  constexpr int TEAM = 64 * TW;
  constexpr int CPT = TEAM / LPC;
  constexpr bool GPF = components_gather_prefetch(P);
  static_assert(LPC >= n2 && CPT >= 1, "lanes per cell");
  static_assert(TW == 1 || TPB == 1, "block-wide barrier needs one team per block");
  using L = LdsLayout<n, LPC>;
  extern __shared__ __attribute__((aligned(16))) double lds[];

  const int tid = threadIdx.x;
  const int team_in_block = tid / TEAM;
  const int t = tid - team_in_block * TEAM;
  const int c = t / LPC, ab = t - c * LPC;
  const uint32_t blk = (blockIdx.x & 7u) * a.teams_per_xcd + (blockIdx.x >> 3);
  const uint32_t team = blk * TPB + team_in_block;
  const uint64_t cell_raw = (uint64_t)a.cell_begin + (uint64_t)team * CPT + c;
  const bool active = (ab < n2) && (c < CPT) && (team < a.n_teams) && (cell_raw < a.cell_end);
  const uint64_t cell = cell_raw < a.cell_end ? cell_raw : (uint64_t)a.cell_end - 1;
  const int abm = ab < n2 ? ab : ab % n2;
  const int a_ = abm % n, b_ = abm / n;
  double *T = lds + (team_in_block * CPT + (c < CPT ? c : 0)) * L::CS;
#define TL(f, k, j, i) T[(f) * (n * L::PS) + (k) * L::PS + (j) * L::RS + (i)]

  uint32_t idx[n];
  const uint32_t *l2g_c = a.l2g + cell * n3 + abm;
#pragma unroll
  for (int k = 0; k < n; ++k) idx[k] = l2g_c[k * n2];
  const double *cf = a.coef + cell * a.cell_stride;
  double S[6][n];
#pragma unroll
  for (int pl = 0; pl < 6; ++pl) load_pencil<n>(cf + pl * a.plane_stride, abm, S[pl]);
  double u[n];
#pragma unroll
  for (int k = 0; k < n; ++k) u[k] = a.src[idx[k]];

  for (uint32_t comp = 0; comp < ca.n_components; ++comp) {
    if constexpr (!GPF) {
// ... 246 lines not shown
#ifndef BP5_PINGPONG_P5
#define BP5_PINGPONG_P5 0
#endif
#ifndef BP5_PINGPONG_P8
#define BP5_PINGPONG_P8 1
#endif
constexpr bool block_pingpong(int degree) { return degree == 2 ? BP5_PINGPONG_P2 != 0 : degree == 5 ? BP5_PINGPONG_P5 != 0 : degree == 8 ? BP5_PINGPONG_P8 != 0 : false; }

template <int n, int LPC, bool PP>
struct BlockLayout {
  using B = LdsLayout<n, LPC>;
  static constexpr int RS = B::RS, PS = B::PS, CS = B::CS, ONE = n * PS + 3, SLOT = (PP ? 2 : 1) * ONE;
};
template <> struct BlockLayout<9, 81, true> { static constexpr int RS = 9, PS = 81, CS = 3 * 9 * 81 + 1, ONE = 732, SLOT = 1465; };
template <> struct BlockLayout<3, 9, true> { static constexpr int RS = 4, PS = 19, CS = 3 * 3 * 19 + 1, ONE = 60, SLOT = 121; };
template <> struct BlockLayout<6, 36, false> { static constexpr int RS = 7, PS = 42, CS = 3 * 6 * 42 + 1, ONE = 252, SLOT = 252; };

constexpr int BLOCK_MAX_RUNS = 128;
constexpr uint32_t BLOCK_DOF_MASK = 0x3fffffffu, BLOCK_DOF_CONSTRAINED = 0x40000000u;
constexpr int PARTIAL_STRIDE = 8192;
constexpr int BLOCK_LATTICE_WORDS = 64;
constexpr int BLOCK_CARRY_MAX = 225;
constexpr int BLOCK_PACK_OFF_BITS = 9;
constexpr int BLOCK_PACK_MAX_RUNS = 1 << (16 - BLOCK_PACK_OFF_BITS);
static_assert(BLOCK_PACK_MAX_RUNS <= BLOCK_MAX_RUNS, "the LDS run table holds every packable run");
struct BlockPlan {
  const uint32_t *pass_cell;
  const uint32_t *pass_off;
  const uint32_t *off;
  const uint32_t *dofs;
  const uint16_t *pos;
  const uint32_t *gidx;
  const uint16_t *packed;
  const uint32_t *lattice;
  const uint16_t *cell_pos;
  const uint8_t *cell_round;
  const uint8_t *blk_rounds;
  double *partial;
  uint32_t n_blocks, n_wg;
  uint32_t blk_begin;
  const uint32_t *wg_block;
  uint32_t n_parts;
  unsigned long long *signal;
  const uint32_t *run_off;
  const uint32_t *runs;
  uint32_t max_list;
  uint32_t carry;
  unsigned long long *stamps;
  const double *cg_r;
  double *dot_partials;
  uint32_t dot_col0;
  uint32_t n_owned;
  const int *cg_state;
};

template <int n, bool AFFINE, int NPL = 6, bool ROLL = false, typename MT = double>
struct PassRegs {
  uint16_t ps[n];
  double u[n];
  MT S[(AFFINE || ROLL) ? 1 : NPL][ROLL ? 1 : n];
  double Gc[AFFINE ? 6 : 1];
  uint32_t idx[n];
  uint32_t ent;
  uint32_t mask;
  uint32_t cpos;
  int round;
  bool active;
};

__device__ __forceinline__ unsigned long long stamp_now()
{
  unsigned long long t;
  __builtin_amdgcn_sched_barrier(0);
  asm volatile("s_memtime %0\n\ts_waitcnt lgkmcnt(0)" : "=s"(t)::"memory");
  __builtin_amdgcn_sched_barrier(0);
  return t;
}
#ifndef BP5_PRIO_Q
#define BP5_PRIO_Q -1
#endif
#ifndef BP5_PRIO_I
#define BP5_PRIO_I -1
#endif
#ifndef BP5_PRIO_A
#define BP5_PRIO_A -1
#endif
#ifndef BP5_PRIO_END
#define BP5_PRIO_END -1
#endif
#define BP5_PRIO_PHASE(k) if constexpr ((k) >= 0) __builtin_amdgcn_s_setprio((k) < 0 ? 0 : (k));
#define BP5_STAMP(slot)                                                                                            \
  if constexpr (ABL & BLK_STAMPS) {                                                                                \
    const unsigned long long now_ = stamp_now();                                                                   \
    ph[slot] += now_ - tprev;                                                                                      \
    tprev = now_;                                                                                                  \
  }

#ifndef BP5_WAVE_PACK
#define BP5_WAVE_PACK 1
#endif
template <int P, bool COLL, int LPC, int SCATTER, int ABL>
struct BlockPass {
  static constexpr int n = P + 1, n2 = n * n, n3 = n2 * n;
  static constexpr int TEAM = 256;
  static constexpr int CPT = TEAM / LPC;
  static constexpr bool AFFINE = (ABL & BLK_AFFINE) != 0;
  static constexpr bool SINGLE = (ABL & BLK_SINGLE) != 0;
// ... 663 lines not shown
#define BP5_WG_PER_CU_P2 4
#endif
template <int P, int ABL>
constexpr int block_wg_per_cu()
{
  if (!(ABL & BLK_SINGLE) || (ABL & BLK_HELM) || BP5_ROLL_TWO(ABL) || P > 4) return 2;
  if (P == 1 && !(ABL & BLK_HANG) && !(ABL & BLK_AFFINE)) return BP5_WG_PER_CU_P1;
  if (P == 2 && BP5_WAVE_PACK != 0 && !(ABL & BLK_HANG) && !(ABL & BLK_AFFINE)) return BP5_WG_PER_CU_P2;
  return 3;
}
#ifndef BP5_SETPRIO
#define BP5_SETPRIO 3
#endif
#ifndef BP5_SETPRIO_WO
#define BP5_SETPRIO_WO 3
#endif
#define BP5_PRIO_ON (BP::LATT || (ABL & BLK_HELM) != 0)
#define BP5_PRIO_HI if constexpr (BP5_SETPRIO != 0 && BP5_PRIO_ON) __builtin_amdgcn_s_setprio(BP5_SETPRIO);
#define BP5_PRIO_LO if constexpr (BP5_SETPRIO != 0 && BP5_PRIO_ON) __builtin_amdgcn_s_setprio(0);
#define BP5_PRIO_WO_HI if constexpr (BP5_SETPRIO_WO != 0 && BP5_PRIO_ON) __builtin_amdgcn_s_setprio(BP5_SETPRIO_WO);
#define BP5_PRIO_WO_LO if constexpr (BP5_SETPRIO_WO != 0 && BP5_PRIO_ON) __builtin_amdgcn_s_setprio(0);
template <int P, bool COLL, int LPC, int SCATTER, int ABL = 0>
__global__ void __launch_bounds__(256, (block_wg_per_cu<P, ABL>())) apply_block_kernel(ApplyArgs a, BlockPlan bp, ShapeArg<P + 1> sh)
{
  using BP = BlockPass<P, COLL, LPC, SCATTER, ABL>;
  constexpr int n = P + 1, n2 = n * n;
  constexpr int TEAM = 256;
  constexpr int CPT = TEAM / LPC;
  static_assert(LPC >= n2 && CPT >= 1, "lanes per cell");
  extern __shared__ __attribute__((aligned(16))) double lds[];
  double *acc = lds + CPT * BP::TILE_CS;

  const int t = threadIdx.x;
  constexpr int CW = 64 / LPC;
  const int c = BP::WPACK ? (((t & 63) < CW * LPC) ? (t >> 6) * CW + (t & 63) / LPC : CPT) : t / LPC;
  const int ab = BP::WPACK ? (t & 63) % LPC : t - c * LPC;
  const uint32_t w = (blockIdx.x & 7u) * (bp.n_wg >> 3) + (blockIdx.x >> 3);
  constexpr bool DOTS = (ABL & BLK_FUSE) != 0;
  static_assert(!DOTS || (((ABL & BLK_RUNS) != 0) && ((ABL & BLK_SEQ) != 0) && SCATTER == SC_OWNER_SET), "fused dot products: run-length write-out, sequential tiles, overwrite mode");
  double ds[4] = {0.0, 0.0, 0.0, 0.0};
  auto signal_part_done = [&](bool stores_pending) {
    if (stores_pending) { lds_drain(); __syncthreads(); }
    if (t == 0) {
      if (stores_pending) __builtin_amdgcn_fence(__ATOMIC_RELEASE, "agent");
      __hip_atomic_fetch_add(bp.signal, 1ull, __ATOMIC_RELAXED, __HIP_MEMORY_SCOPE_AGENT);
    }
  };
  if constexpr (DOTS) {
    if (bp.cg_state[0]) {
      if (bp.signal) signal_part_done(false);
      return;
    }
  }
  const uint32_t ba0 = bp.wg_block[w], ba1 = bp.wg_block[w + 1];
  const uint32_t bb0 = bp.n_parts > 1 ? bp.wg_block[bp.n_wg + 1 + w] : 0u, bb1 = bp.n_parts > 1 ? bp.wg_block[bp.n_wg + 1 + w + 1] : 0u;
  const uint32_t nba = ba1 - ba0, b1 = nba + (bb1 - bb0);
  if (b1 == 0) {
    if constexpr (DOTS) { if (t < 7) bp.dot_partials[t * PARTIAL_STRIDE + bp.dot_col0 + blockIdx.x] = 0.0; }
    if (bp.signal) signal_part_done(false);
    return;
  }
  if (bp.signal && nba == 0) signal_part_done(false);
  const uint32_t pa0 = bp.pass_off[ba0], npa = bp.pass_off[ba1] - pa0, pb0 = bp.pass_off[bb0];
  auto blk = [&](uint32_t vb) -> uint32_t { return vb < nba ? ba0 + vb : bb0 + (vb - nba); };
  uint32_t b = 0;
  uint32_t pb = blk(0);
  uint32_t gp = 0;
  const uint32_t gp_end = npa + (bp.pass_off[bb1] - pb0);
  uint32_t boundary = bp.pass_off[pb + 1] - bp.pass_off[pb];
  uint32_t o0 = bp.off[pb];
  int m = (int)(bp.off[pb + 1] - o0);
  int n_rounds = bp.blk_rounds[pb];
  constexpr bool RUNS = (ABL & BLK_RUNS) != 0;
  constexpr bool STAGE = BP::STAGE;
  double *const staged = acc + bp.max_list;
  uint32_t *const run_tab = reinterpret_cast<uint32_t *>(acc + (STAGE ? 2 : 1) * (size_t)bp.max_list);
  uint32_t *const lat_tab = run_tab + 4 * BLOCK_MAX_RUNS;
  constexpr bool use_lattice = BP::LATT;
  uint32_t lat_word = 0;
  constexpr bool CARRY = (ABL & BLK_CARRY) != 0;
  static_assert(!CARRY || (BP::LATT && RUNS), "face carry: lattice blocks with run tables");
  double *const carry_buf = reinterpret_cast<double *>(lat_tab + 2 * BLOCK_LATTICE_WORDS);
  bool c_carried = false;
  uint32_t c_in_w = 0, c_out_w = 0;
  auto c_in_at = [&](int i) { return (uint32_t)(i - (int)(c_in_w & 0xffffu)) < (c_in_w >> 16); };
  auto c_out_at = [&](int i) { return (uint32_t)(i - (int)(c_out_w & 0xffffu)) < (c_out_w >> 16); };
  uint32_t r0 = RUNS ? bp.run_off[pb] : 0u;
  int n_runs = RUNS ? (int)(bp.run_off[pb + 1] - r0) : 0;
  uint32_t run_slot = 0, run_dof = 0;
  const bool lane_ok = (ab < n2) && (c < CPT);
  const int abm = ab < n2 ? ab : ab % n2;
  const int slot = c < CPT ? c : 0;
  const int a_ = abm % n, b_ = abm / n;
  double *T = lds + slot * BP::TILE_CS;

  for (int i = t; i < (int)bp.max_list; i += TEAM) acc[i] = 0.0;
  __syncthreads();

  auto entry = [&](uint32_t pass) {
    const uint32_t v = pass < gp_end ? pass : gp_end - 1;
    return bp.pass_cell[(uint64_t)(v < npa ? pa0 + v : pb0 + (v - npa)) * CPT + slot];
  };
  auto enter_block = [&](const uint32_t *rt_, int n_runs_, int m_) {
    int r = 0;
    for (int i = 2 * t; i < m_; i += 2 * TEAM) {
      while (r + 1 < n_runs_ && (int)rt_[r + 1] <= i) ++r;
      const uint32_t g = (rt_[BLOCK_MAX_RUNS + r] & BLOCK_DOF_MASK) + (uint32_t)(i - (int)rt_[r]);
      const bool run_ends = r + 1 < n_runs_ && (int)rt_[r + 1] == i + 1;
      if (i + 1 < m_ && !run_ends) {
        const bp5_d2u v = *reinterpret_cast<const bp5_d2u *>(a.src + g);
        staged[i] = v.x;
        staged[i + 1] = v.y;
      } else {
        staged[i] = a.src[g];
        if (i + 1 < m_) staged[i + 1] = a.src[rt_[BLOCK_MAX_RUNS + r + 1] & BLOCK_DOF_MASK];
      }
    }
  };

  unsigned long long ph[8] = {0, 0, 0, 0, 0, 0, 0, 0}, tprev = 0;
  if constexpr (ABL & BLK_STAMPS) tprev = stamp_now();
  typename BP::R A, B;
  double Sroll[BP::ROLL ? BP::NPL : 1][BP::ROLL ? n : 1];
  A.ent = entry(gp);
  B.ent = entry(gp + 1);
  BP::issue_loads(a, bp, A, abm, lane_ok, true);
  if constexpr (BP::ROLL) BP::issue_metric_roll(a, A.ent, abm, Sroll);
  if constexpr (BP::PACK) {
    uint32_t *const rt0 = run_tab + (b & 1u) * (2 * BLOCK_MAX_RUNS);
    if (t < n_runs) {
      rt0[t] = bp.runs[2 * (r0 + t)];
      rt0[BLOCK_MAX_RUNS + t] = bp.runs[2 * (r0 + t) + 1];
    }
    if constexpr (use_lattice) { if (t < BLOCK_LATTICE_WORDS) lat_tab[(b & 1u) * BLOCK_LATTICE_WORDS + t] = bp.lattice[(uint64_t)pb * BLOCK_LATTICE_WORDS + t]; }
    __syncthreads();
    if constexpr (STAGE) {
      enter_block(rt0, n_runs, m);
      __syncthreads();
    }
    BP::decode_and_gather(a, A, rt0, staged, use_lattice ? lat_tab + (b & 1u) * BLOCK_LATTICE_WORDS : nullptr, a_, b_);
  } else
    BP::issue_gather(a, A);

  constexpr int MAXW = (ABL & BLK_SINGLE) ? 1 : 6;
  uint32_t gl[MAXW];
  uint32_t nx_boundary = 0, nx_o0 = 0, nx_o1 = 0, nx_r0 = 0, nx_r1 = 0;
  int nx_rounds = 1;
  auto prefetch_list = [&]() {
    if (gp + 1 == boundary && b + 1 < b1) {
      const uint32_t p1 = blk(b + 1);
      nx_boundary = boundary + (bp.pass_off[p1 + 1] - bp.pass_off[p1]);
      nx_o0 = bp.off[p1];
      nx_o1 = bp.off[p1 + 1];
      nx_rounds = bp.blk_rounds[p1];
      if constexpr (RUNS) {
        nx_r0 = bp.run_off[p1];
        nx_r1 = bp.run_off[p1 + 1];
      }
      if constexpr (use_lattice) { if (t < BLOCK_LATTICE_WORDS) lat_word = bp.lattice[(uint64_t)p1 * BLOCK_LATTICE_WORDS + t]; }
    }
    if (gp + 1 == boundary) {
      if constexpr (BP::PACK) {
        if (b + 1 < b1) {
          if (t < (int)(nx_r1 - nx_r0)) {
            run_slot = bp.runs[2 * (nx_r0 + t)];
            run_dof = bp.runs[2 * (nx_r0 + t) + 1];
          }
        }
      } else if constexpr (RUNS) {
        if (t < n_runs) {
          run_slot = bp.runs[2 * (r0 + t)];
          run_dof = bp.runs[2 * (r0 + t) + 1];
        }
      } else {
#pragma unroll
        for (int r = 0; r < MAXW; ++r) gl[r] = (t + r * TEAM < m) ? bp.dofs[o0 + t + r * TEAM] : 0u;
      }
    }
  };
  auto carry_mark = [&](int i, uint32_t g) -> uint32_t {
    if constexpr (CARRY) { if (c_in_at(i)) return g | 0x80000000u; }
    return g;
  };
  auto emit = [&](int i, uint32_t g, double ri = 0.0) {
    double v = acc[i];
    acc[i] = 0.0;
    if constexpr (CARRY) {
      if (c_in_at(i)) v += carry_buf[((b + 1) & 1u) * BLOCK_CARRY_MAX + (i - (int)(c_in_w & 0xffffu))];
      if (c_out_at(i)) { carry_buf[(b & 1u) * BLOCK_CARRY_MAX + (i - (int)(c_out_w & 0xffffu))] = v; return; }
    }
    if (g & 0x80000000u) {
      const uint32_t gi = g & BLOCK_DOF_MASK;
      if constexpr (DOTS) {
        double vi = v;
        if (g & BLOCK_DOF_CONSTRAINED) {
          vi = a.src[gi];
          if (gi < bp.n_owned) ds[0] = __builtin_fma(vi, vi - v, ds[0]);
        }
        __builtin_nontemporal_store(vi, a.dst + gi);
        if (gi < bp.n_owned) { ds[1] = __builtin_fma(vi, vi, ds[1]); ds[2] = __builtin_fma(ri, vi, ds[2]); ds[3] = __builtin_fma(ri, ri, ds[3]); }
      } else if constexpr (ABL & 16) { if (v == 1.2345e300) a.dst[gi] = v; }
      else if constexpr (SCATTER == SC_OWNER_SET || SCATTER == SC_OWNER_SET_ATOMIC) {
        if constexpr (ABL & 65536) a.dst[gi] = v;
        else __builtin_nontemporal_store(v, a.dst + gi);
      }
      else a.dst[gi] += v;
    } else {
      if constexpr (ABL & 16) { if (v == 1.2345e300) bp.partial[o0 + i] = v; }
      else if constexpr (SCATTER == SC_OWNER_SET_ATOMIC || SCATTER == SC_OWNER_ADD_ATOMIC) atomic_add_f64(a.dst + (g & BLOCK_DOF_MASK), v);
      else if constexpr (ABL & 65536) bp.partial[o0 + i] = v;
      else __builtin_nontemporal_store(v, bp.partial + o0 + i);
    }
// ... 10 lines not shown
      if (c_out_at(i)) {
        double *cb = carry_buf + (b & 1u) * BLOCK_CARRY_MAX + (i - (int)(c_out_w & 0xffffu));
        cb[0] = v0; cb[1] = v1;
        return;
      }
    }
    if (g & 0x80000000u) {
      const uint32_t gi = g & BLOCK_DOF_MASK;
      double *d = a.dst + gi;
      if constexpr (DOTS) {
        double w0 = v0, w1 = v1;
        if (g & BLOCK_DOF_CONSTRAINED) {
          const bp5_d2u pv = *reinterpret_cast<const bp5_d2u *>(a.src + gi);
          w0 = pv.x; w1 = pv.y;
          if (gi < bp.n_owned) ds[0] = __builtin_fma(w0, w0 - v0, ds[0]);
          if (gi + 1 < bp.n_owned) ds[0] = __builtin_fma(w1, w1 - v1, ds[0]);
        }
        __builtin_nontemporal_store(bp5_d2u{w0, w1}, reinterpret_cast<bp5_d2u *>(d));
        if (gi < bp.n_owned) { ds[1] = __builtin_fma(w0, w0, ds[1]); ds[2] = __builtin_fma(rv.x, w0, ds[2]); ds[3] = __builtin_fma(rv.x, rv.x, ds[3]); }
        if (gi + 1 < bp.n_owned) { ds[1] = __builtin_fma(w1, w1, ds[1]); ds[2] = __builtin_fma(rv.y, w1, ds[2]); ds[3] = __builtin_fma(rv.y, rv.y, ds[3]); }
      } else if constexpr (SCATTER == SC_OWNER_SET || SCATTER == SC_OWNER_SET_ATOMIC) {
        if constexpr (ABL & 65536) { d[0] = v0; d[1] = v1; }
        else __builtin_nontemporal_store(bp5_d2u{v0, v1}, reinterpret_cast<bp5_d2u *>(d));
      } else {
        const bp5_d2u o = *reinterpret_cast<const bp5_d2u *>(d);
        *reinterpret_cast<bp5_d2u *>(d) = bp5_d2u{o.x + v0, o.y + v1};
      }
    } else {
      if constexpr (SCATTER == SC_OWNER_SET_ATOMIC || SCATTER == SC_OWNER_ADD_ATOMIC) {
        atomic_add_f64(a.dst + (g & BLOCK_DOF_MASK), v0);
        atomic_add_f64(a.dst + (g & BLOCK_DOF_MASK) + 1, v1);
      } else if constexpr (ABL & 65536) { bp.partial[o0 + i] = v0; bp.partial[o0 + i + 1] = v1; }
      else __builtin_nontemporal_store(bp5_d2u{v0, v1}, reinterpret_cast<bp5_d2u *>(bp.partial + o0 + i));
    }
  };
  auto finish_pass = [&]() {
    if (gp + 1 == boundary) {
      uint32_t *const rt = run_tab + (b & 1u) * (2 * BLOCK_MAX_RUNS);
      if constexpr (BP::PACK) {
        if (b + 1 < b1) {
          uint32_t *const rn = run_tab + ((b + 1) & 1u) * (2 * BLOCK_MAX_RUNS);
          if (t < (int)(nx_r1 - nx_r0)) {
            rn[t] = run_slot;
            rn[BLOCK_MAX_RUNS + t] = run_dof;
          }
          if constexpr (use_lattice) { if (t < BLOCK_LATTICE_WORDS) lat_tab[((b + 1) & 1u) * BLOCK_LATTICE_WORDS + t] = lat_word; }
        }
      } else if constexpr (RUNS) {
        if (t < n_runs) {
          rt[t] = run_slot;
          rt[BLOCK_MAX_RUNS + t] = run_dof;
        }
      }
      __syncthreads();
      BP5_PRIO_WO_HI
      if constexpr (CARRY) {
        const uint32_t *lt = lat_tab + (b & 1u) * BLOCK_LATTICE_WORDS;
        uint32_t wo = 0u, wi = 0u;
        if (bp.carry) { wo = lt[55]; wi = lt[56]; }
        c_out_w = (b + 1 < b1 && b + 1 != nba) ? (uint32_t)__builtin_amdgcn_readfirstlane((int)wo) : 0u;
        c_in_w = c_carried ? (uint32_t)__builtin_amdgcn_readfirstlane((int)wi) : 0u;
      }
      if constexpr (DOTS) {
        constexpr int NW = 5;
        const bool has_r = bp.cg_r != nullptr;
        int r = 0;
        for (int base = 2 * t; base < m; base += NW * 2 * TEAM) {
          uint32_t g0[NW], g1[NW];
          int kind[NW];
          bp5_d2u rv[NW];
#pragma unroll
          for (int j = 0; j < NW; ++j) {
            const int i = base + j * 2 * TEAM;
            g0[j] = g1[j] = 0u;
            kind[j] = 0;
            rv[j] = bp5_d2u{0.0, 0.0};
            if (i < m) {
              while (r + 1 < n_runs && (int)rt[r + 1] <= i) ++r;
              g0[j] = carry_mark(i, rt[BLOCK_MAX_RUNS + r] + (uint32_t)(i - (int)rt[r]));
              const bool run_ends = r + 1 < n_runs && (int)rt[r + 1] == i + 1;
              const uint32_t gi = g0[j] & BLOCK_DOF_MASK;
              if (i + 1 < m && !run_ends) {
                kind[j] = 1;
                if (has_r && (g0[j] & 0x80000000u)) rv[j] = *reinterpret_cast<const bp5_d2u *>(bp.cg_r + gi);
              } else {
                kind[j] = 2;
                if (has_r && (g0[j] & 0x80000000u)) rv[j].x = bp.cg_r[gi];
                if (i + 1 < m) {
                  kind[j] = 3;
                  g1[j] = carry_mark(i + 1, rt[BLOCK_MAX_RUNS + r + 1]);
                  if (has_r && (g1[j] & 0x80000000u)) rv[j].y = bp.cg_r[g1[j] & BLOCK_DOF_MASK];
                }
              }
            }
          }
#pragma unroll
          for (int j = 0; j < NW; ++j) {
            const int i = base + j * 2 * TEAM;
            if (kind[j] == 1) emit2(i, g0[j], rv[j]);
            else if (kind[j]) {
              emit(i, g0[j], rv[j].x);
              if (kind[j] == 3) emit(i + 1, g1[j], rv[j].y);
            }
          }
        }
      } else if constexpr (RUNS && !(ABL & 1)) {
        int r = 0;
        for (int i = 2 * t; i < m; i += 2 * TEAM) {
          while (r + 1 < n_runs && (int)rt[r + 1] <= i) ++r;
          const uint32_t g = carry_mark(i, rt[BLOCK_MAX_RUNS + r] + (uint32_t)(i - (int)rt[r]));
          const bool run_ends = r + 1 < n_runs && (int)rt[r + 1] == i + 1;
          if (i + 1 < m && !run_ends) emit2(i, g);
          else {
            emit(i, g);
            if (i + 1 < m) emit(i + 1, carry_mark(i + 1, rt[BLOCK_MAX_RUNS + r + 1]));
          }
        }
      }
      if constexpr (!RUNS && !(ABL & 1)) {
#pragma unroll
        for (int r = 0; r < MAXW; ++r) {
          const int i = t + r * TEAM;
          if (i < m) emit(i, gl[r]);
        }
        for (int base = t + MAXW * TEAM; base < m; base += 8 * TEAM) {
          uint32_t g8[8];
#pragma unroll
          for (int r = 0; r < 8; ++r) g8[r] = (base + r * TEAM < m) ? bp.dofs[o0 + base + r * TEAM] : 0u;
#pragma unroll
          for (int r = 0; r < 8; ++r)
            if (base + r * TEAM < m) emit(base + r * TEAM, g8[r]);
        }
      }
      if constexpr (CARRY) c_carried = c_out_w != 0u;
      BP5_PRIO_WO_LO
      ++b;
      if (bp.signal && b == nba) signal_part_done(true);
      if (b < b1) {
        boundary = nx_boundary;
        o0 = nx_o0;
        m = (int)(nx_o1 - nx_o0);
        n_rounds = nx_rounds;
        if constexpr (RUNS) {
          r0 = nx_r0;
          n_runs = (int)(nx_r1 - nx_r0);
        }
        if constexpr (STAGE) {
          enter_block(run_tab + (b & 1u) * (2 * BLOCK_MAX_RUNS), n_runs, m);
          __syncthreads();
        }
      }
    }
    ++gp;
  };

  while (gp < gp_end) {
    prefetch_list();
    BP5_PRIO_HI BP::issue_loads(a, bp, B, abm, lane_ok, gp + 1 < gp_end); BP5_PRIO_LO
    const uint32_t entA2 = entry(gp + 2);
    BP::run(a, sh, A, B, T, acc, a_, b_, n_rounds, abm, ph, tprev, ds[0], Sroll);
    finish_pass();
    BP5_STAMP(6)
    if (gp >= gp_end) break;
    BP5_PRIO_HI if constexpr (BP::PACK) BP::decode_and_gather(a, B, run_tab + (b & 1u) * (2 * BLOCK_MAX_RUNS), staged, use_lattice ? lat_tab + (b & 1u) * BLOCK_LATTICE_WORDS : nullptr, a_, b_);
    A.ent = entA2;
    prefetch_list();
    BP5_PRIO_HI BP::issue_loads(a, bp, A, abm, lane_ok, gp + 1 < gp_end); BP5_PRIO_LO
    const uint32_t entB2 = entry(gp + 2);
    BP::run(a, sh, B, A, T, acc, a_, b_, n_rounds, abm, ph, tprev, ds[0], Sroll);
    finish_pass();
    BP5_STAMP(6)
    BP5_PRIO_HI if constexpr (BP::PACK) { if (gp < gp_end) BP::decode_and_gather(a, A, run_tab + (b & 1u) * (2 * BLOCK_MAX_RUNS), staged, use_lattice ? lat_tab + (b & 1u) * BLOCK_LATTICE_WORDS : nullptr, a_, b_); } BP5_PRIO_LO
    B.ent = entB2;
  }
  if constexpr (DOTS) {
    __syncthreads();
    double *red = lds;
#pragma unroll
    for (int k = 0; k < 4; ++k) {
      double v = ds[k];
#pragma unroll
      for (int off = 32; off > 0; off >>= 1) v += __shfl_down(v, off, 64);
      if ((t & 63) == 0) red[k * 4 + (t >> 6)] = v;
    }
    __syncthreads();
    if (t < 7) {
      const int k = t < 4 ? t : (t == 4 ? 2 : t == 5 ? 1 : 3);
      bp.dot_partials[t * PARTIAL_STRIDE + bp.dot_col0 + blockIdx.x] = (red[k * 4] + red[k * 4 + 1]) + (red[k * 4 + 2] + red[k * 4 + 3]);
    }
  }
  if constexpr (ABL & BLK_STAMPS) {
    if (t == 0) {
#pragma unroll
      for (int k = 0; k < 8; ++k) bp.stamps[(uint64_t)w * 16 + k] = ph[k];
      bp.stamps[(uint64_t)w * 16 + 8] = gp_end;
    }
  }
}

template <int n>
struct Cell3 {
  static constexpr int n2 = n * n, n3 = n * n * n;
  template <bool TR>
  static __device__ double tensor3(const double *Mx, const double *My, const double *Mz, const double *src, double *t1,
                                   double *t2, int i, int j, int k)
  {
    double acc = 0.0;
    for (int m = 0; m < n; ++m) acc += (TR ? Mx[m * n + i] : Mx[i * n + m]) * src[m + n * (j + n * k)];
    t1[i + n * (j + n * k)] = acc;
// ... 739 lines not shown
  }
  __syncthreads();
  if (threadIdx.x < K) {
    double s = 0.0;
#pragma unroll
    for (int w = 0; w < VB / 64; ++w) s += red[threadIdx.x][w];
    partials[threadIdx.x * PARTIAL_STRIDE + blockIdx.x] = s;
  }
}

template <int K>
__global__ void __launch_bounds__(VB) finalize_kernel(const double *partials, int nblk, double *out, const int *state)
{
  if (state && state[0]) return;
  __shared__ double red[VB];
  for (int k = blockIdx.x; k < K; k += gridDim.x) {
    double s = 0.0;
    for (int i = threadIdx.x; i < nblk; i += VB) s += partials[k * PARTIAL_STRIDE + i];
    red[threadIdx.x] = s;
    __syncthreads();
    for (int off = VB / 2; off > 0; off >>= 1) {
      if ((int)threadIdx.x < off) red[threadIdx.x] += red[threadIdx.x + off];
      __syncthreads();
    }
    if (threadIdx.x == 0) out[k] = red[0];
    __syncthreads();
  }
}

static __global__ void __launch_bounds__(VB) dot_kernel(const double *x, const double *y, size_t n, double *partials)
{
  double acc[1] = {0.0};
  const size_t stride = (size_t)gridDim.x * VB * 2;
  for (size_t i = ((size_t)blockIdx.x * VB + threadIdx.x) * 2; i < n; i += stride) {
    if (i + 1 < n) {
      const double2 a = *reinterpret_cast<const double2 *>(x + i), b = *reinterpret_cast<const double2 *>(y + i);
      acc[0] += a.x * b.x + a.y * b.y;
    } else
      acc[0] += x[i] * y[i];
  }
  block_reduce_store<1>(acc, partials);
}

static __global__ void __launch_bounds__(VB) count_nonzero_kernel(const double *x, size_t n, double *partials)
{
  double acc[1] = {0.0};
  const size_t stride = (size_t)gridDim.x * VB;
  for (size_t i = (size_t)blockIdx.x * VB + threadIdx.x; i < n; i += stride) acc[0] += (x[i] == 0.0) ? 0.0 : 1.0;
  block_reduce_store<1>(acc, partials);
}

enum { SC_GH = 0, SC_DH, SC_GG, SC_GDG, SC_ALPHA, SC_BETA, SC_ALPHA_OLD, SC_BETA_OLD, SC_RES, SC_RES0, SC_TOL, SC_R0 ,
       SC_COUNT = SC_R0 + 7 };
enum { ST_DONE = 0, ST_ITER, ST_PENDING, ST_MAXIT, ST_BREAKDOWN, ST_COUNT };

static __global__ void copy_constrained_components_kernel(const uint32_t *cdofs, uint32_t n, const double *src, double *dst, size_t ld)
{
  const uint32_t i = blockIdx.x * blockDim.x + threadIdx.x;
  if (i < n) { const size_t c = cdofs[i] + blockIdx.y * ld; dst[c] = src[c]; }
}

template <bool GDG>
__global__ void __launch_bounds__(VB) cg_init_kernel(const double *b, const double *diag, double *x, double *g, double *d, size_t n, size_t ld,
                                                     double *partials)
{
  const size_t o = blockIdx.y * ld;
  b += o; x += o; g += o; d += o;
  double acc[GDG ? 2 : 1] = {};
  const size_t stride = (size_t)gridDim.x * VB;
  for (size_t i = (size_t)blockIdx.x * VB + threadIdx.x; i < n; i += stride) {
    if constexpr (GDG) {
      const double gi = -b[i], hi = diag ? diag[i] * gi : gi;
      x[i] = 0.0; g[i] = gi; d[i] = -hi;
      acc[0] += gi * gi; acc[1] += gi * hi;
    } else {
      const double gi = -b[i];
      x[i] = 0.0; g[i] = gi;
      acc[0] += gi * gi;
    }
  }
  block_reduce_store<GDG ? 2 : 1>(acc, partials + blockIdx.y * gridDim.x);
}
static __global__ void cg_init_control_kernel(double *sc, int *st)
{
  sc[SC_RES0] = sc[SC_RES] = sqrt(sc[SC_GG]);
  sc[SC_GH] = sc[SC_GDG];
  st[ST_ITER] = 0; st[ST_PENDING] = 0; st[ST_BREAKDOWN] = 0;
  st[ST_DONE] = (sc[SC_RES] <= sc[SC_TOL]) ? 1 : 0;
}
template <bool COPY>
__global__ void __launch_bounds__(VB) cg_dh_kernel(const double *d, double *h, size_t n, size_t ld, double *partials, const int *st, const uint32_t *cbits)
{
  if (st[ST_DONE]) return;
  d += blockIdx.y * ld; h += blockIdx.y * ld;
  double acc[1] = {0.0};
  const size_t stride = (size_t)gridDim.x * VB * 2;
  for (size_t i = ((size_t)blockIdx.x * VB + threadIdx.x) * 2; i < n; i += stride) {
    if constexpr (COPY) {
      const uint32_t cb = (cbits[i >> 5] >> (i & 31)) & 3u;
      if (i + 1 < n) {
        const double2 a = *reinterpret_cast<const double2 *>(d + i);
        double2 b = *reinterpret_cast<double2 *>(h + i);
        if (cb) {
          if (cb & 1u) b.x = a.x;
          if (cb & 2u) b.y = a.y;
          *reinterpret_cast<double2 *>(h + i) = b;
        }
// ... 48 lines not shown
  block_reduce_store<GDG ? 2 : 1>(acc, partials + blockIdx.y * gridDim.x);
}
static __global__ void cg_control_kernel(double *sc, int *st)
{
  if (st[ST_DONE]) return;
  const double dh = sc[SC_DH];
  if (!(dh == dh) || dh == 0.0) { st[ST_BREAKDOWN] = 1; st[ST_DONE] = 1; return; }
  const double res = sqrt(sc[SC_GG]);
  sc[SC_RES] = res;
  sc[SC_ALPHA] = sc[SC_GH] / dh;
  const int it = ++st[ST_ITER];
  if (res <= sc[SC_TOL] || it >= st[ST_MAXIT]) { st[ST_DONE] = 1; return; }
  sc[SC_BETA] = sc[SC_GDG] / sc[SC_GH];
  sc[SC_GH] = sc[SC_GDG];
}
template <bool Z, bool FIRST>
__global__ void __launch_bounds__(VB) cg_direction_kernel(double *d, const double *g, const double *diag, size_t n, size_t ld, const double *sc,
                                                          const int *st)
{
  if (st[ST_DONE]) return;
  d += blockIdx.y * ld; g += blockIdx.y * ld;
  const double beta = FIRST ? 0.0 : sc[SC_BETA];
  const size_t stride = (size_t)gridDim.x * VB * 2;
  for (size_t i = ((size_t)blockIdx.x * VB + threadIdx.x) * 2; i < n; i += stride) {
    if (i + 1 < n) {
      double2 dv = FIRST ? double2{0.0, 0.0} : *reinterpret_cast<double2 *>(d + i);
      const double2 gv = *reinterpret_cast<const double2 *>(g + i);
      dv.x = FIRST ? -gv.x : beta * dv.x - (!Z && diag ? diag[i] * gv.x : gv.x);
      dv.y = FIRST ? -gv.y : beta * dv.y - (!Z && diag ? diag[i + 1] * gv.y : gv.y);
      *reinterpret_cast<double2 *>(d + i) = dv;
    } else
      d[i] = FIRST ? -g[i] : beta * d[i] - (!Z && diag ? diag[i] * g[i] : g[i]);
  }
}

template <int MODE>
__device__ __forceinline__ void cgm_update_one(double &p, double &r, const double v, double &x, const double di, const bool done,
                                               const bool epi_odd, const double alpha, const double beta, const double aob)
{
  if (done) {
    if (epi_odd) x = fma(alpha, p, x);
    else x = fma(aob, di * r, fma(alpha + aob, p, x));
    return;
  }
  if (MODE == 0) {
    p = -(di * r);
  } else {
    if (MODE == 2) x = fma(aob, di * r, fma(alpha + aob, p, x));
    const double rn = fma(alpha, v, r);
    r = rn;
    p = fma(beta, p, -(di * rn));
  }
}
template <int MODE, int U = 2, bool ZV = false, bool NTX = false>
__global__ void __launch_bounds__(VB) cgm_update_kernel(double *p, double *r, typename std::conditional<ZV, double, const double>::type *v, double *x,
                                                       const double *diag, size_t n, const double *sc, const int *st)
{
  const bool done = st[ST_DONE];
  if (done && !st[ST_PENDING]) return;
  const double alpha = sc[SC_ALPHA], beta = sc[SC_BETA];
  const double aob = (MODE == 2 || done) ? sc[SC_ALPHA_OLD] / sc[SC_BETA_OLD] : 0.0;
  const bool epi_odd = done && (st[ST_ITER] & 1);
  const bool touch_x = done || MODE == 2, touch_rp = !done;
  const size_t stride = (size_t)gridDim.x * VB * 2 * U;
  for (size_t base = ((size_t)blockIdx.x * VB * U + threadIdx.x) * 2; base < n; base += stride) {
    double2 pv[U], rv[U], vv[U], xv[U];
#pragma unroll
    for (int u = 0; u < U; ++u) {
      const size_t i = base + (size_t)u * VB * 2;
      pv[u] = rv[u] = vv[u] = xv[u] = double2{0, 0};
      if (i + 1 < n) {
        pv[u] = *reinterpret_cast<double2 *>(p + i);
        rv[u] = *reinterpret_cast<double2 *>(r + i);
        if (MODE != 0 && !done) {
          if constexpr (NTX) { const bp5_d2u t = __builtin_nontemporal_load(reinterpret_cast<const bp5_d2u *>(v + i)); vv[u] = double2{t.x, t.y}; }
          else vv[u] = *reinterpret_cast<const double2 *>(v + i);
        }
        if (touch_x) {
          if constexpr (NTX) { const bp5_d2u t = __builtin_nontemporal_load(reinterpret_cast<const bp5_d2u *>(x + i)); xv[u] = double2{t.x, t.y}; }
          else xv[u] = *reinterpret_cast<double2 *>(x + i);
        }
      } else if (i < n) {
        pv[u].x = p[i]; rv[u].x = r[i];
        if (MODE != 0 && !done) vv[u].x = v[i];
        if (touch_x) xv[u].x = x[i];
      }
    }
#pragma unroll
    for (int u = 0; u < U; ++u) {
      const size_t i = base + (size_t)u * VB * 2;
      if (i >= n) continue;
      const bool pair = i + 1 < n;
      const double d0 = diag ? diag[i] : 1.0, d1 = (diag && pair) ? diag[i + 1] : 1.0;
      cgm_update_one<MODE>(pv[u].x, rv[u].x, vv[u].x, xv[u].x, d0, done, epi_odd, alpha, beta, aob);
      if (pair) cgm_update_one<MODE>(pv[u].y, rv[u].y, vv[u].y, xv[u].y, d1, done, epi_odd, alpha, beta, aob);
      if (pair) {
        if (touch_rp) {
          *reinterpret_cast<double2 *>(p + i) = pv[u];
          if (MODE != 0) *reinterpret_cast<double2 *>(r + i) = rv[u];
        }
        if (touch_x) {
          if constexpr (NTX) __builtin_nontemporal_store(bp5_d2u{xv[u].x, xv[u].y}, reinterpret_cast<bp5_d2u *>(x + i));
          else *reinterpret_cast<double2 *>(x + i) = xv[u];
        }
        if constexpr (ZV) { if (MODE != 0 && !done) *reinterpret_cast<double2 *>(v + i) = double2{0.0, 0.0}; }
      } else {
        if (touch_rp) { p[i] = pv[u].x; if (MODE != 0) r[i] = rv[u].x; }
        if (touch_x) x[i] = xv[u].x;
        if constexpr (ZV) { if (MODE != 0 && !done) v[i] = 0.0; }
      }
    }
  }
}
template <int MODE>
__global__ void __launch_bounds__(256) cgm_pack_updated_kernel(const uint32_t *idx, uint32_t n, const double *p, const double *r, const double *v,
                                                             const double *diag, const double *sc, const int *st, double *buf)
{
  const uint32_t i = blockIdx.x * 256u + threadIdx.x;
  if (i >= n) return;
  const uint32_t g = idx[i];
  double pi = p[g];
  if (!st[ST_DONE]) {
    double ri = r[g], xi = 0.0;
    const double vi = MODE != 0 ? v[g] : 0.0;
    cgm_update_one<MODE>(pi, ri, vi, xi, diag ? diag[g] : 1.0, false, false, sc[SC_ALPHA], sc[SC_BETA], 0.0);
  }
  buf[i] = pi;
}

static __global__ void __launch_bounds__(VB) cgm_dots_kernel(const double *p, const double *r, double *v, const double *diag, size_t n,
                                                     const int *st, double *partials, const uint32_t *cbits)
{
  if (st[ST_DONE]) return;
  double acc[7] = {0, 0, 0, 0, 0, 0, 0};
  auto one = [&](double pi, double ri, double vi, double di) {
    acc[0] += pi * vi; acc[1] += vi * vi; acc[2] += ri * vi; acc[3] += ri * ri;
    acc[4] += ri * di * vi; acc[5] += vi * di * vi; acc[6] += ri * di * ri;
  };
  const size_t stride = (size_t)gridDim.x * VB * 2;
  for (size_t i = ((size_t)blockIdx.x * VB + threadIdx.x) * 2; i < n; i += stride) {
    const uint32_t cb = cbits ? (cbits[i >> 5] >> (i & 31)) & 3u : 0u;
    if (i + 1 < n) {
      const double2 pv = *reinterpret_cast<const double2 *>(p + i), rv = *reinterpret_cast<const double2 *>(r + i);
      double2 vv = *reinterpret_cast<const double2 *>(v + i);
      if (cb) {
        if (cb & 1u) vv.x = pv.x;
        if (cb & 2u) vv.y = pv.y;
        *reinterpret_cast<double2 *>(v + i) = vv;
      }
      one(pv.x, rv.x, vv.x, diag ? diag[i] : 1.0);
      one(pv.y, rv.y, vv.y, diag ? diag[i + 1] : 1.0);
    } else {
      double vi = v[i];
      if (cb & 1u) { vi = p[i]; v[i] = vi; }
      one(p[i], r[i], vi, diag ? diag[i] : 1.0);
    }
  }
  block_reduce_store<7>(acc, partials);
}
static __global__ void cgm_control_kernel(double *sc, int *st);
__device__ __forceinline__ void cgm_control_step(double *sc, int *st)
{
  if (st[ST_DONE]) { st[ST_PENDING] = 0; return; }
  const double *R = sc + SC_R0;
  if (!(R[0] == R[0]) || R[0] == 0.0) { st[ST_BREAKDOWN] = 1; st[ST_DONE] = 1; return; }
  sc[SC_ALPHA_OLD] = sc[SC_ALPHA];
  sc[SC_BETA_OLD] = sc[SC_BETA];
  const double alpha = R[6] / R[0];
  sc[SC_ALPHA] = alpha;
  const double r2 = R[3] + 2.0 * alpha * R[2] + alpha * alpha * R[1];
  const double res = sqrt(r2 > 0.0 ? r2 : 0.0);
  sc[SC_RES] = res;
  const int it = ++st[ST_ITER];
  if (res <= sc[SC_TOL] || it >= st[ST_MAXIT]) { st[ST_DONE] = 1; st[ST_PENDING] = 1; return; }
  sc[SC_BETA] = alpha * (R[4] + alpha * R[5]) / R[6];
}
constexpr int FIN4_THREADS = 1024;
template <bool CONTROL>
__global__ void __launch_bounds__(FIN4_THREADS) cgm_finalize4_kernel(const double *partials, int nblk, double *sc, int *st)
{
  if (st[ST_DONE]) {
    if (CONTROL && threadIdx.x == 0) cgm_control_step(sc, st);
    return;
  }
  __shared__ double red[16];
  const int wave = threadIdx.x >> 6, lane = threadIdx.x & 63;
  const int k = wave >> 2, l = ((wave & 3) << 6) | lane;
  const double *row = partials + k * PARTIAL_STRIDE;
  double s0 = 0.0, s1 = 0.0, s2 = 0.0, s3 = 0.0;
  for (int i = l; i < nblk; i += 1024) {
    const double a0 = row[i], a1 = i + 256 < nblk ? row[i + 256] : 0.0, a2 = i + 512 < nblk ? row[i + 512] : 0.0, a3 = i + 768 < nblk ? row[i + 768] : 0.0;
    s0 += a0; s1 += a1; s2 += a2; s3 += a3;
  }
  double s = (s0 + s1) + (s2 + s3);
#pragma unroll
  for (int off = 32; off > 0; off >>= 1) s += __shfl_down(s, off, 64);
  if (lane == 0) red[wave] = s;
  __syncthreads();
  double *out = sc + SC_R0;
  if (threadIdx.x < 4) {
    const int r = threadIdx.x;
    const double t = (red[4 * r] + red[4 * r + 1]) + (red[4 * r + 2] + red[4 * r + 3]);
    out[r] = t;
    if (r == 1) out[5] = t;
    if (r == 2) out[4] = t;
    if (r == 3) out[6] = t;
  }
  if constexpr (CONTROL) {
    __syncthreads();
    if (threadIdx.x == 0) cgm_control_step(sc, st);
  }
}

static __global__ void cgm_control_kernel(double *sc, int *st) { cgm_control_step(sc, st); }

static __global__ void __launch_bounds__(VB) cgm_init_kernel(const double *b, double *x, double *r, double *p, double *v, const double *diag, size_t n,
                                                     double *partials, bool zero_v)
{
  double acc[2] = {0.0, 0.0};
  const size_t stride = (size_t)gridDim.x * VB;
  for (size_t i = (size_t)blockIdx.x * VB + threadIdx.x; i < n; i += stride) {
    const double ri = -b[i], di = diag ? diag[i] : 1.0;
    x[i] = 0.0; r[i] = ri; p[i] = -(di * ri);
    if (zero_v) v[i] = 0.0;
    acc[0] += ri * ri;
  }
  acc[1] = acc[0];
  block_reduce_store<2>(acc, partials);
}
static __global__ void cgm_init_control_kernel(double *sc, int *st)
{
  sc[SC_RES0] = sc[SC_RES] = sqrt(sc[SC_GG]);
  sc[SC_ALPHA] = sc[SC_BETA] = sc[SC_ALPHA_OLD] = sc[SC_BETA_OLD] = 0.0;
  st[ST_ITER] = 0; st[ST_PENDING] = 0; st[ST_BREAKDOWN] = 0;
  st[ST_DONE] = (sc[SC_RES] <= sc[SC_TOL]) ? 1 : 0;
}

static __global__ void cg_record_kernel(const double *sc, const int *st, double *hist, int cap)
{
  const int k = st[ST_ITER];
  if (k < 1 || k > cap || st[ST_BREAKDOWN]) return;
  hist[2 * k - 2] = sc[SC_ALPHA];
  hist[2 * k - 1] = st[ST_DONE] ? 0.0 : sc[SC_BETA];
}

template <int FORM, bool DIAG, bool NT>
__global__ void __launch_bounds__(VB) chebyshev_step_kernel(double *x_new, const double *x, const double *x_old, const double *src, const double *t,
                                                            const double *diag, size_t n, double f1, double f2)
{
  auto load = [](const double *p, bool nt) -> double2 {
    if (nt) { const bp5_d2u v = __builtin_nontemporal_load(reinterpret_cast<const bp5_d2u *>(p)); return double2{v.x, v.y}; }
    return *reinterpret_cast<const double2 *>(p);
  };
  const size_t stride = (size_t)gridDim.x * VB * 2;
  for (size_t i = ((size_t)blockIdx.x * VB + threadIdx.x) * 2; i < n; i += stride) {
    if (i + 1 < n) {
      const double2 s = load(src + i, false);
      const double2 dg = DIAG ? load(diag + i, false) : double2{1.0, 1.0};
      double2 r;
      if constexpr (FORM == 0) {
        r.x = f2 * (dg.x * s.x);
        r.y = f2 * (dg.y * s.y);
      } else {
        const double2 tv = load(t + i, NT), xv = load(x + i, false);
        const double2 xo = FORM == 1 ? load(x_old + i, NT) : double2{0.0, 0.0};
        const double2 f1x = FORM == 3 ? double2{0.0, 0.0} : double2{f1 * (xv.x - xo.x), f1 * (xv.y - xo.y)};
        r.x = xv.x + f1x.x + f2 * (dg.x * (s.x - tv.x));
        r.y = xv.y + f1x.y + f2 * (dg.y * (s.y - tv.y));
      }
      *reinterpret_cast<double2 *>(x_new + i) = r;
    } else {
      const double dg = DIAG ? diag[i] : 1.0;
      if constexpr (FORM == 0) x_new[i] = f2 * (dg * src[i]);
      else {
        const double xv = x[i], xo = FORM == 1 ? x_old[i] : 0.0;
        x_new[i] = xv + (FORM == 3 ? 0.0 : f1 * (xv - xo)) + f2 * (dg * (src[i] - t[i]));
      }
    }
  }
}

template <int NF, int NC>
struct MgShape {
  static constexpr int F3 = NF * NF * NF, C3 = NC * NC * NC;
  static constexpr int CPB = F3 >= 256 ? 1 : 256 / F3;
  static constexpr int WORDS = (F3 + 31) / 32;
  static constexpr int LDS = F3 + NC * NF * NF + NC * NC * NF;
// ... 620 lines not shown
```

deal-and-ceed-on-gpu_amd/matrix_free.py:

```python
import ctypes as C

import numpy as np

from . import _lib
from ._lib import BP5Error, CG_MERGED, CG_PLAIN, COEF_ONE, QUAD_GAUSS


def _torch():
    import torch
    return torch


def _ptr(t, n_min=0):
    torch = _torch()
    if t is None:
        return None
    if not (isinstance(t, torch.Tensor) and t.is_cuda and t.dtype == torch.float64 and t.is_contiguous()):
        raise BP5Error(1, "expected a contiguous float64 CUDA tensor")
    if t.numel() < n_min:
        raise BP5Error(1, f"vector has {t.numel()} entries, need {n_min}")
    return C.c_void_p(t.data_ptr())


class Communicator:
# ... 72 lines not shown
    def handle(self):
        if not self._h:
            raise BP5Error(1, "MatrixFree.reinit has not been called")
        return self._h

    def close(self):
        if self._h:
            _lib.lib().bp5_mf_destroy(self._h)
            self._h = None

    def __del__(self):
        try:
            self.close()
        except Exception:
            pass

    def synchronize(self):
        _lib.check(_lib.lib().bp5_mf_sync(self.handle))

    def set_geometry_mode(self, mode):
        _lib.check(_lib.lib().bp5_mf_set_geometry_mode(self.handle, int(mode)))

    def set_overlap(self, mode=True):
        _lib.check(_lib.lib().bp5_mf_set_overlap(self.handle, int(mode)))

    def set_cg_fusion(self, on=True):
        _lib.check(_lib.lib().bp5_mf_set_cg_fusion(self.handle, 1 if on else 0))

    def set_apply_variant(self, v):
        _lib.check(_lib.lib().bp5_mf_set_apply_variant(self.handle, int(v)))

    def set_operator(self, op):
        _lib.check(_lib.lib().bp5_mf_set_operator(self.handle, int(op)))

    METRIC_PRECISION = {"float64": 0, "float32": 1}

    def set_metric_precision(self, precision):
        if precision not in self.METRIC_PRECISION:
            raise BP5Error(1, f"metric precision must be 'float64' or 'float32', not {precision!r}")
        _lib.check(_lib.lib().bp5_mf_set_metric_precision(self.handle, self.METRIC_PRECISION[precision]))

    def get_metric_precision(self):
        v = C.c_int()
        _lib.check(_lib.lib().bp5_mf_get_metric_precision(self.handle, C.byref(v)))
        return "float32" if v.value == 1 else "float64"

    def set_block_workgroups(self, n):
        _lib.check(_lib.lib().bp5_mf_set_block_workgroups(self.handle, int(n)))

    def set_streaming(self, policy):
        _lib.check(_lib.lib().bp5_mf_set_streaming(self.handle, int(policy)))

    TUNE = {"lattice_indices": 0, "early_gather": 1, "combine_signal": 2, "boundary_first": 3, "fold_small": 4, "update_unroll": 5,
            "update_flat": 6, "update_nt": 7, "combine_wg_per_cu": 8, "interior_stores": 9, "ghost_combine_on_comm": 10, "face_carry": 11}

    def set_tuning(self, knob, value):
        _lib.check(_lib.lib().bp5_mf_set_tuning(self.handle, int(self.TUNE.get(knob, knob)), int(value)))

    def get_tuning(self, knob):
        v = C.c_int()
        _lib.check(_lib.lib().bp5_mf_get_tuning(self.handle, int(self.TUNE.get(knob, knob)), C.byref(v)))
        return v.value

    def wait_value_available(self):
        v = C.c_int()
        _lib.check(_lib.lib().bp5_mf_wait_value_available(self.handle, C.byref(v)))
        return bool(v.value)

    def block_plan_info(self):
        nb, mr, pk = C.c_uint32(), C.c_uint32(), C.c_int()
        _lib.check(_lib.lib().bp5_mf_block_plan_info(self.handle, C.byref(nb), C.byref(mr), C.byref(pk)))
        return nb.value, mr.value, bool(pk.value)

    def block_plan_lattice(self):
        n = C.c_uint32()
        _lib.check(_lib.lib().bp5_mf_block_plan_lattice(self.handle, C.byref(n)))
        return n.value

    def block_plan_carry(self):
        a, b, c = C.c_uint32(), C.c_uint32(), C.c_uint32()
        _lib.check(_lib.lib().bp5_mf_block_plan_carry(self.handle, C.byref(a), C.byref(b), C.byref(c)))
        return a.value, b.value, c.value

    def get_apply_variant(self):
        v = C.c_int()
        _lib.check(_lib.lib().bp5_mf_get_apply_variant(self.handle, C.byref(v)))
        return v.value

    def initialize_dof_vector(self, vec=None):
        torch = _torch()
        return torch.zeros(self.n_local, dtype=torch.float64, device=f"cuda:{self.device}")

    def initialize_block_vector(self, n_components):
        torch = _torch()
        if not 1 <= int(n_components) <= _lib.MAX_COMPONENTS:
            raise BP5Error(1, f"n_components must be 1 .. {_lib.MAX_COMPONENTS}, not {n_components!r}")
        return torch.zeros((int(n_components), self.n_local + (self.n_local & 1)), dtype=torch.float64, device=f"cuda:{self.device}")

    def coef_size(self):
        n = C.c_size_t()
        _lib.check(_lib.lib().bp5_mf_coef_size(self.handle, C.byref(n)))
        return n.value

    def evaluate_coefficients(self, coef=None):
        torch = _torch()
        if coef is None:
            coef = torch.empty(max(self.coef_size(), 1), dtype=torch.float64, device=f"cuda:{self.device}")
# ... 572 lines not shown
```

include/bp5.h:

```cpp
#ifndef BP5_H
#define BP5_H

#include <stddef.h>
#include <stdint.h>

#ifdef __cplusplus
extern "C" {
#endif

enum {
  BP5_OK = 0,
  BP5_ERR_INVALID = 1,
  BP5_ERR_HIP = 2,
  BP5_ERR_NO_DEVICE = 3,
  BP5_ERR_RCCL = 4,
  BP5_ERR_UNSUPPORTED = 5,
  BP5_ERR_BREAKDOWN = 6,
  BP5_ERR_NO_CONVERGENCE = 7
};
const char *bp5_strerror(int status);
const char *bp5_last_error(void);

enum { BP5_QUAD_GAUSS = 0,
       BP5_QUAD_GLL = 1,
// ... 74 lines not shown
  void *stream;
  uint32_t n_cell_blocks;
  const uint32_t *cell_block_offsets_host;
  const uint32_t *constraint_mask_host;
} bp5_mf_desc;

enum { BP5_HANG_FACE_X = 1, BP5_HANG_FACE_Y = 2, BP5_HANG_FACE_Z = 4,
       BP5_HANG_SIDE_X = 8, BP5_HANG_SIDE_Y = 16, BP5_HANG_SIDE_Z = 32,
       BP5_HANG_HALF_X = 64, BP5_HANG_HALF_Y = 128, BP5_HANG_HALF_Z = 256,
       BP5_HANG_EDGE_X = 512, BP5_HANG_EDGE_Y = 1024, BP5_HANG_EDGE_Z = 2048 };

int bp5_mf_create(const bp5_mf_desc *desc, bp5_mf **out);
int bp5_mf_destroy(bp5_mf *mf);
int bp5_mf_set_stream(bp5_mf *mf, void *hip_stream);
int bp5_mf_sync(bp5_mf *mf);

enum { BP5_OP_POISSON = 0, BP5_OP_HELMHOLTZ = 1, BP5_OP_MASS = 2 };
int bp5_mf_set_operator(bp5_mf *mf, int op);
enum { BP5_METRIC_F64 = 0, BP5_METRIC_F32 = 1 };
int bp5_mf_set_metric_precision(bp5_mf *mf, int precision);
int bp5_mf_get_metric_precision(const bp5_mf *mf, int *precision);
int bp5_mf_coef_size(const bp5_mf *mf, size_t *n_doubles);

int bp5_mf_compute_merged_metric(bp5_mf *mf, double *coef);
enum { BP5_GEOM_MERGED6 = 0, BP5_GEOM_AFFINE = 1 };
int bp5_mf_set_geometry_mode(bp5_mf *mf, int mode);
int bp5_mf_metric_to_reference_layout(bp5_mf *mf, const double *coef, double *coef_ref);

typedef struct {
  const uint32_t *local_to_global;
  const double *inv_jacobian;
  const double *JxW;
  const double *q_points;
  const uint32_t *constraint_mask;
  uint32_t n_cells, padding_length, row_start;
  int use_coloring;
} bp5_mf_data;
int bp5_mf_get_data(bp5_mf *mf, int color, bp5_mf_data *out);

int bp5_apply(bp5_mf *mf, const double *coef, const double *src, double *dst, int zero_dst);
int bp5_apply_cells(bp5_mf *mf, const double *coef, const double *src, double *dst, uint32_t cell_begin,
                    uint32_t cell_end);
int bp5_copy_constrained(bp5_mf *mf, const double *src, double *dst);
int bp5_set_constrained(bp5_mf *mf, double value, double *dst);

#define BP5_MAX_COMPONENTS 8
int bp5_apply_components(bp5_mf *mf, const double *coef, int n_components, size_t ld, const double *src, double *dst, int zero_dst);

int bp5_mf_set_apply_variant(bp5_mf *mf, int variant);
int bp5_mf_set_block_workgroups(bp5_mf *mf, int max_workgroups);
int bp5_mf_set_streaming(bp5_mf *mf, int policy);
enum { BP5_TUNE_LATTICE_INDICES = 0, BP5_TUNE_EARLY_GATHER = 1, BP5_TUNE_COMBINE_SIGNAL = 2, BP5_TUNE_BOUNDARY_FIRST = 3,
       BP5_TUNE_FOLD_SMALL = 4, BP5_TUNE_UPDATE_UNROLL = 5, BP5_TUNE_UPDATE_FLAT = 6, BP5_TUNE_UPDATE_NT = 7, BP5_TUNE_COMBINE_WG_PER_CU = 8,
       BP5_TUNE_INTERIOR_STORES = 9, BP5_TUNE_GHOST_COMBINE_ON_COMM = 10, BP5_TUNE_FACE_CARRY = 11, BP5_TUNE_COUNT = 12 };
int bp5_mf_set_tuning(bp5_mf *mf, int knob, int value);
int bp5_mf_get_tuning(const bp5_mf *mf, int knob, int *value);
int bp5_mf_wait_value_available(bp5_mf *mf, int *available);
int bp5_mf_block_plan_info(bp5_mf *mf, uint32_t *n_blocks, uint32_t *max_runs, int *packed_indices);
int bp5_mf_block_plan_lattice(bp5_mf *mf, uint32_t *n_lattice_blocks);
int bp5_mf_block_plan_carry(bp5_mf *mf, uint32_t *n_faces, uint32_t *n_shared, uint32_t *n_shared_last_launch);
int bp5_mf_get_apply_variant(bp5_mf *mf, int *effective);

int bp5_compute_diagonal(bp5_mf *mf, const double *coef, double *diag, int invert);

int bp5_assemble_rhs(bp5_mf *mf, double *b);
int bp5_l2_norm_solution(bp5_mf *mf, const double *u, double *result_host);

int bp5_vec_fill(bp5_mf *mf, double *v, double value, size_t n);
int bp5_vec_axpy(bp5_mf *mf, double *y, double a, const double *x, size_t n);
int bp5_vec_equ(bp5_mf *mf, double *y, double a, const double *x, size_t n);
int bp5_vec_sadd(bp5_mf *mf, double *y, double s, double a, const double *x, size_t n);
int bp5_vec_dot(bp5_mf *mf, const double *x, const double *y, size_t n, double *result_host);
int bp5_vec_l2_norm(bp5_mf *mf, const double *x, size_t n, double *result_host);
int bp5_vec_all_zero(bp5_mf *mf, const double *x, size_t n, int *result_host);

typedef struct bp5_comm bp5_comm;
#define BP5_UNIQUE_ID_BYTES 128
int bp5_comm_unique_id(char *id_host );
int bp5_comm_create(const char *id_host, int rank, int n_ranks, bp5_comm **out);
int bp5_comm_destroy(bp5_comm *comm);
int bp5_mf_set_comm(bp5_mf *mf, bp5_comm *comm);
int bp5_comm_allreduce_sum(bp5_mf *mf, double *buf, size_t n);
int bp5_halo_gather_start(bp5_mf *mf, double *v);
int bp5_halo_gather_finish(bp5_mf *mf, double *v);
int bp5_halo_scatter_add_start(bp5_mf *mf, double *v);
int bp5_halo_scatter_add_finish(bp5_mf *mf, double *v);
int bp5_halo_gather(bp5_mf *mf, double *v);
int bp5_halo_scatter_add(bp5_mf *mf, double *v);
int bp5_halo_zero_ghosts(bp5_mf *mf, double *v);
int bp5_mf_set_overlap(bp5_mf *mf, int mode);
int bp5_apply_distributed(bp5_mf *mf, const double *coef, double *src, double *dst, int zero_dst);

int bp5_halo_gather_components(bp5_mf *mf, int n_components, size_t ld, double *v);
int bp5_halo_scatter_add_components(bp5_mf *mf, int n_components, size_t ld, double *v);
int bp5_halo_zero_ghosts_components(bp5_mf *mf, int n_components, size_t ld, double *v);
int bp5_apply_components_distributed(bp5_mf *mf, const double *coef, int n_components, size_t ld, double *src, double *dst, int zero_dst);

enum { BP5_CG_PLAIN = 0,
       BP5_CG_MERGED = 1   };

typedef struct {
  int variant;
  int max_iter;
  double abs_tol;
  int check_every;
  int profile;
} bp5_cg_params;
// ... 99 lines not shown
```

Baseline: 29.70 billion.

## Fuse CG vector update for brick-interior DoFs into the block operator kernel

When every cell block has lattice indices and brick interiors are numbered contiguously first, the CG p/r/x update for those interior DoFs is done inside the block apply kernel, just before each block is gathered. A separate rest kernel updates only the remaining DoFs. The aim is to drop one full streaming pass over p, r, v and x for most of the vector, saving HBM traffic. The cost is extra setup logic, a hold flag in the control state, and more work and register pressure in the apply kernel. It only applies to single-rank p=4 Poisson runs with no ghosts and large problem sizes.

Result: faster. 30.95 billion (median of 6 runs) (+4.2%).

```diff
diff --git a/deal-and-ceed-on-gpu_amd/csrc/bp5_device.hip b/deal-and-ceed-on-gpu_amd/csrc/bp5_device.hip
--- a/deal-and-ceed-on-gpu_amd/csrc/bp5_device.hip
+++ b/deal-and-ceed-on-gpu_amd/csrc/bp5_device.hip
@@ -777,6 +777,35 @@
   BP5_TRY(upload_combine_tables(start, dof0, soff, slots, out));
   out->n_shared_owned = owned;
   return BP5_OK;
+}
+
+static uint32_t interior_runs_cover(const bp5_mf *mf, int p, const TeamPlanHost &h, const std::vector<uint32_t> &lat)
+{
+  const size_t ng = h.off.size() - 1;
+  std::vector<std::pair<uint32_t, uint32_t>> runs(ng);
+  bool ok = true;
+#pragma omp parallel for schedule(dynamic, 16) reduction(&& : ok)
+  for (int64_t g = 0; g < (int64_t)ng; ++g) {
+    const uint32_t *row = lat.data() + (size_t)g * BLOCK_LATTICE_WORDS;
+    const uint32_t hdr = row[54];
+    if (!(hdr >> 31)) { ok = false; continue; }
+    const uint32_t len = ((hdr & 255u) * p - 1u) * (((hdr >> 8) & 255u) * p - 1u) * (((hdr >> 16) & 255u) * p - 1u), dof = row[27 + 13], slot = row[13];
+    runs[g] = {dof, len};
+    if (!len || (uint64_t)h.off[g] + slot + len > h.off[g + 1]) { ok = false; continue; }
+    const uint32_t *l = h.dofs.data() + h.off[g] + slot;
+    for (uint32_t k = 0; k < len; ++k)
+      if (l[k] != ((dof + k) | 0x80000000u)) { ok = false; break; }
+  }
+  if (!ok) return 0;
+  std::sort(runs.begin(), runs.end());
+  uint64_t end = 0;
+  for (const auto &r : runs) {
+    if (r.first != end) return 0;
+    end += r.second;
+  }
+  if (end == 0 || end > mf->n_owned) return 0;
+  for (uint64_t i = 0; i < end; ++i) if (mf->h_constrained[i]) return 0;
+  return (uint32_t)end;
 }
 
 int get_plan_raw(bp5_mf *mf, int key, bp5_mf::DevPlan **dpo, int default_block)
@@ -858,6 +887,7 @@
         if (!faces.empty()) mark_carry_faces(h, faces, run_off, runs, lat, dp);
         BP5_TRY(upload(&dp.lattice, lat.data(), lat.size()));
         BP5_TRY(upload(&dp.cell_pos, cpos.data(), cpos.size()));
+        if (dp.n_lattice_blocks == (uint32_t)(h.off.size() - 1)) dp.upd_n_int = interior_runs_cover(mf, mf->degree, h, lat);
       } else
         dp.n_lattice_blocks = 0;
     } else
@@ -1482,6 +1512,7 @@
   mf->tune[BP5_TUNE_INTERIOR_STORES] = env_int("BP5_INTERIOR_STORES", 1) != 0;
   mf->tune[BP5_TUNE_GHOST_COMBINE_ON_COMM] = env_int("BP5_GHOST_COMBINE_ON_COMM", 0) != 0;
   mf->tune[BP5_TUNE_FACE_CARRY] = env_int("BP5_FACE_CARRY", 1) != 0;
+  { const int v = env_int("BP5_FUSED_UPDATE", -1); mf->tune[BP5_TUNE_FUSED_UPDATE] = (v >= -1 && v <= 1) ? v : -1; }
 }
 extern "C" int bp5_mf_set_tuning(bp5_mf *mf, int knob, int value)
 {
@@ -1492,6 +1523,9 @@
       break;
     case BP5_TUNE_UPDATE_NT:
       if (value < -1 || value > 1) return fail(BP5_ERR_INVALID, "BP5_TUNE_UPDATE_NT: -1, 0 or 1");
+      break;
+    case BP5_TUNE_FUSED_UPDATE:
+      if (value < -1 || value > 1) return fail(BP5_ERR_INVALID, "BP5_TUNE_FUSED_UPDATE: -1, 0 or 1");
       break;
     case BP5_TUNE_COMBINE_WG_PER_CU:
       if (value < 0 || value > 32) return fail(BP5_ERR_INVALID, "BP5_TUNE_COMBINE_WG_PER_CU: 0 ... 32");
@@ -1966,6 +2000,9 @@
   bool two_parts = false;
   bool gather_in_flight = false;
   bool dst_prezeroed = false, copies_dirichlet = false;
+  int upd_mode = 0;
+  double *upd_x = nullptr;
+  const double *upd_diag = nullptr;
   bool phase_on = false;
   int phase_it = 0;
   uint8_t phase_recorded[bp5_mf::PhaseProfile::MAX_ITERS] = {};
@@ -2113,7 +2150,7 @@
   BP5_TRY(prof.mark(1));
   if (prof.on) call.mark_event = mf->ev_pool[prof.used + 2];
   FuseState fuse;
-  if (fusing) { fuse.p = src; fuse.r = fuse_r; call.fuse = &fuse; }
+  if (fusing) { fuse.p = src; fuse.r = fuse_r; fuse.upd_mode = ss.upd_mode; fuse.upd_x = ss.upd_x; fuse.upd_diag = ss.upd_diag; call.fuse = &fuse; }
   call.overwrite = zero;
   BP5_TRY(launch_apply(mf, call, coef, src, dst));
   if (fusing) *n_cols = fuse.n_cols;
@@ -2196,6 +2233,7 @@
   bool fused_dots = false;
   bool fold_small = false;
   bool prezero = false;
+  uint32_t fused_update = 0;
   int schedule = 0;
 };
 static int plan_operator(bp5_mf *mf, bool own_operator, bool fusable, SolveState &ss, OperatorPlan &op)
@@ -2214,6 +2252,13 @@
       if (mf->overlap == 1 && !split) op.fused_dots = false;
       late = op.fused_dots && mf->overlap == 2 && (dp->n_shared == 0 || dp->cr_tile);
     }
+  }
+  if (op.fused_dots && !op.dist && !mf->comm && mf->n_ghost == 0 && mf->degree == 4 && mf->tune[BP5_TUNE_FUSED_UPDATE] != 0 &&
+      mf->operator_kind == BP5_OP_POISSON && !mf->has_hanging && !mf->overint() && effective_variant(mf, 0, mf->n_cells) == 56) {
+    bp5_mf::DevPlan *dp = nullptr;
+    BP5_TRY(get_plan_raw(mf, -block_cpt(mf), &dp));
+    const bool by_size = mf->tune[BP5_TUNE_FUSED_UPDATE] < 0;
+    if (dp->lattice && dp->n_lattice_blocks == dp->n_groups && dp->upd_n_int >= 2 && (!by_size || mf->n_local() > STREAMING_MAX_DOFS)) op.fused_update = dp->upd_n_int;
   }
   ss.exchange = split ? EXCHANGE_BOUNDARY_FIRST : late ? EXCHANGE_GHOST_ROWS_FIRST : EXCHANGE_NONE;
   ss.two_parts = op.fused_dots && op.dist && split_possible;
@@ -2373,7 +2418,8 @@
   hipLaunchKernelGGL(finalize_kernel<2>, dim3(2), dim3(VB), 0, s, mf->d_partials, grid1, mf->d_sc + SC_GG, (const int *)nullptr);
   KERNEL_CHECK();
   BP5_TRY(bp5_comm_allreduce_sum(mf, mf->d_sc + SC_GG, 2));
-  hipLaunchKernelGGL(cgm_init_control_kernel, dim3(1), dim3(1), 0, s, mf->d_sc, mf->d_st);
+  const size_t n_first = fused && !user ? (size_t)(op.fused_update & ~1u) : 0;
+  hipLaunchKernelGGL(cgm_init_control_kernel, dim3(1), dim3(1), 0, s, mf->d_sc, mf->d_st, n_first ? 1 : 0);
   KERNEL_CHECK();
   const int unroll = mf->tune[BP5_TUNE_UPDATE_UNROLL];
   const int gridu = stream_grid_flat(mf, n, 2 * unroll);
@@ -2388,6 +2434,16 @@
 #undef BP5_UPD_U
 #undef BP5_UPD
   };
+  const int gridr = n > n_first ? stream_grid_flat(mf, n - n_first, 2 * unroll) : 0;
+  auto launch_update_rest = [&](int mode) {
+    if (!gridr) return;
+#define BP5_UPR(M, U, NT) hipLaunchKernelGGL((cgm_update_rest_kernel<M, U, NT>), dim3(gridr), dim3(VB), 0, s, d, g, h, x, diag, n_first, n - n_first, mf->d_sc, mf->d_st)
+#define BP5_UPR_U(M, NT) do { if (unroll == 1) BP5_UPR(M, 1, NT); else if (unroll == 2) BP5_UPR(M, 2, NT); else BP5_UPR(M, 4, NT); } while (0)
+    if (streaming) { if (mode == 1) BP5_UPR_U(1, true); else BP5_UPR_U(2, true); return; }
+    if (mode == 1) BP5_UPR_U(1, false); else BP5_UPR_U(2, false);
+#undef BP5_UPR_U
+#undef BP5_UPR
+  };
   const bool early_gather_enabled = mf->tune[BP5_TUNE_EARLY_GATHER] != 0;
   const bool early_gather = fused && dist_solve && early_gather_enabled;
   auto gather_under_update = [&](int mode) -> int {
@@ -2406,7 +2462,10 @@
     const int mode = it == 1 ? 0 : it % 2 == 0 ? 1 : 2;
     BP5_TRY(phase_mark(mf, ss, 0));
     if (early_gather) { BP5_TRY(gather_under_update(mode)); ss.gather_in_flight = true; }
-    if (mode != 0) launch_update(mode);
+    if (mode != 0) {
+      if (n_first) launch_update_rest(mode); else launch_update(mode);
+    }
+    ss.upd_mode = n_first ? mode : 0; ss.upd_x = x; ss.upd_diag = diag;
     KERNEL_CHECK();
     BP5_TRY(phase_mark(mf, ss, 1));
     const bool one_launch = fused && !mf->comm;
@@ -2441,6 +2500,7 @@
   }
   if (prm->max_iter > 0) {
     launch_update(1);
+    if (n_first) HIP_TRY(hipMemsetD32Async((hipDeviceptr_t)(mf->d_st + ST_HOLD), 0, 1, s));
     hipLaunchKernelGGL(cgm_control_kernel, dim3(1), dim3(1), 0, s, mf->d_sc, mf->d_st);
     KERNEL_CHECK();
   }
diff --git a/deal-and-ceed-on-gpu_amd/csrc/bp5_device.hpp b/deal-and-ceed-on-gpu_amd/csrc/bp5_device.hpp
--- a/deal-and-ceed-on-gpu_amd/csrc/bp5_device.hpp
+++ b/deal-and-ceed-on-gpu_amd/csrc/bp5_device.hpp
@@ -89,7 +89,7 @@
   uint64_t signal_target = 0;
   int wait_value_ok = -1;
   int can_wait_value = -1;
-  int tune[BP5_TUNE_COUNT] = {1, 1, 0, 1, 1, 1, 1, -1, 16, 1, 0, 1};
+  int tune[BP5_TUNE_COUNT] = {1, 1, 0, 1, 1, 1, 1, -1, 16, 1, 0, 1, -1};
   bool cell_interiors_first = false;
   double *d_partials = nullptr, *d_sc = nullptr, *d_scalar = nullptr;
   int *d_st = nullptr;
@@ -124,6 +124,7 @@
     uint32_t *lattice = nullptr;
     uint16_t *cell_pos = nullptr;
     uint32_t n_lattice_blocks = 0;
+    uint32_t upd_n_int = 0;
     std::vector<double> h_cost;
     std::map<std::tuple<uint32_t, uint32_t, uint32_t, uint32_t>, uint32_t *> *wg_blocks = nullptr;
     uint32_t *cr_start = nullptr, *cr_dof0 = nullptr, *cr_soff = nullptr, *cr_slots = nullptr, *cr_tile = nullptr;
@@ -149,6 +150,9 @@
   const double *p = nullptr, *r = nullptr;
   uint32_t n_cols = 0;
   bool ghosts_zeroed = false;
+  int upd_mode = 0;
+  double *upd_x = nullptr;
+  const double *upd_diag = nullptr;
 };
 enum VariantFamily { VARIANT_PENCIL, VARIANT_TEAM, VARIANT_MARCH, VARIANT_BLOCK, VARIANT_BLOCK_SIBLING, VARIANT_HANGING_PENCIL, VARIANT_OTHER };
 struct VariantInfo {
@@ -470,6 +474,12 @@
     }
   }
   bp.cg_r = call.fuse ? call.fuse->r : nullptr; bp.dot_partials = mf->d_partials; bp.n_owned = mf->n_owned; bp.cg_state = mf->d_st;
+  if constexpr ((ABL & BLK_UPD) != 0) {
+    if (!call.fuse || !call.fuse->upd_mode || !call.fuse->r || !dp->upd_n_int || sub_range || bp.n_parts != 1 || mf->n_ghost)
+      return fail(BP5_ERR_INVALID, "the fused-update build needs a one-rank merged solve on a plan whose brick interiors are numbered first");
+    bp.upd_p = const_cast<double *>(src); bp.upd_r = const_cast<double *>(call.fuse->r); bp.upd_v = dst; bp.upd_x = call.fuse->upd_x;
+    bp.upd_diag = call.fuse->upd_diag; bp.upd_sc = mf->d_sc; bp.upd_mode = (uint32_t)call.fuse->upd_mode; bp.upd_end = dp->upd_n_int & ~1u;
+  }
   bp.stamps = nullptr;
   if (ABL & BLK_STAMPS) {
     if (!mf->d_stamps) HIP_TRY(hipMalloc((void **)&mf->d_stamps, 4096 * 16 * sizeof(unsigned long long)));
@@ -618,7 +628,8 @@
 template <>
 struct DefaultBlockBuilds<4> {
   static constexpr int D = BLK_DEFAULT, F = BLK_FUSE, LATC = BLK_LATT | BLK_CARRY;
-  using list = BuildList<Bld<D | LATC | BLK_NTM, true>, Bld<D | F | LATC | BLK_NTM, true>, Bld<D | LATC>, Bld<D | F | LATC>, Bld<D>, Bld<D | F>,
+  using list = BuildList<Bld<D | F | LATC | BLK_UPD | BLK_NTM>, Bld<D | F | LATC | BLK_UPD>,
+                         Bld<D | LATC | BLK_NTM, true>, Bld<D | F | LATC | BLK_NTM, true>, Bld<D | LATC>, Bld<D | F | LATC>, Bld<D>, Bld<D | F>,
 #ifdef BP5_TIMING_BUILDS
                          Bld<D | BLK_LATT | BLK_NTM | BLK_ROLL, true>, Bld<D | F | BLK_LATT | BLK_NTM | BLK_ROLL, true>, Bld<D | BLK_LATT | BLK_ROLL, true>,
                          Bld<D | F | BLK_LATT | BLK_ROLL, true>,
@@ -660,7 +671,12 @@
   if (dp->packed && variant != 49) {
     want = BLK_DEFAULT | cls | (call.fuse ? BLK_FUSE : 0);
     if (dp->lattice && dp->n_lattice_blocks == dp->n_groups && variant != 48) want |= BLK_LATT | BLK_CARRY;
-    if (streaming_accesses(mf)) want |= BLK_NTM;
+    const bool upd = call.fuse && call.fuse->upd_mode != 0;
+    if (upd) {
+      if (DEG != 4 || !(want & BLK_LATT) || cls != 0) return fail(BP5_ERR_INVALID, "the fused vector update needs the p = 4 lattice build of the Poisson operator");
+      want |= BLK_UPD;
+    }
+    if (upd && mf->streaming < 0 ? true : streaming_accesses(mf)) want |= BLK_NTM;
   } else {
     if (DEG != 4 || cls != 0) return fail(BP5_ERR_UNSUPPORTED, "variant " + std::to_string(variant) + " needs packed indices (<= 128 runs per cell block)");
     if (call.fuse) return fail(BP5_ERR_INVALID, "fused dot products need the packed block kernel");
diff --git a/deal-and-ceed-on-gpu_amd/csrc/bp5_kernels.hpp b/deal-and-ceed-on-gpu_amd/csrc/bp5_kernels.hpp
--- a/deal-and-ceed-on-gpu_amd/csrc/bp5_kernels.hpp
+++ b/deal-and-ceed-on-gpu_amd/csrc/bp5_kernels.hpp
@@ -12,7 +12,7 @@
 };
 
 enum : int {
-  BLK_AFFINE = 1024, BLK_SINGLE = 2048, BLK_STAMPS = 4096, BLK_SEQ = 8192, BLK_RUNS = 16384, BLK_NTM = 32768, BLK_PACK = 262144,
+  BLK_AFFINE = 1024, BLK_SINGLE = 2048, BLK_STAMPS = 4096, BLK_SEQ = 8192, BLK_RUNS = 16384, BLK_NTM = 32768, BLK_UPD = 131072, BLK_PACK = 262144,
   BLK_STAGE = 524288, BLK_FUSE = 1048576, BLK_HANG = 2097152, BLK_LDSADD = 4194304, BLK_HELM = 8388608, BLK_LATT = 16777216,
   BLK_ROLL = 67108864, BLK_CARRY = 268435456,
   BLK_F32M = 536870912,
@@ -1059,6 +1059,7 @@
 }
 
 __device__ __forceinline__ void lds_drain() { asm volatile("s_waitcnt lgkmcnt(0)" ::: "memory"); }
+__device__ __forceinline__ void vmem_drain() { asm volatile("s_waitcnt vmcnt(0)" ::: "memory"); }
 
 struct ComponentArgs {
   uint32_t n_components;
@@ -1411,7 +1412,14 @@
   uint32_t dot_col0;
   uint32_t n_owned;
   const int *cg_state;
+  double *upd_p, *upd_r, *upd_x;
+  const double *upd_v;
+  const double *upd_diag;
+  const double *upd_sc;
+  uint32_t upd_mode;
+  uint32_t upd_end;
 };
+template <int MODE> __device__ __forceinline__ void block_update_run(const BlockPlan &bp, uint32_t lo, uint32_t hi, int t);
 
 template <int n, bool AFFINE, int NPL = 6, bool ROLL = false, typename MT = double>
 struct PassRegs {
@@ -2181,6 +2189,16 @@
       return;
     }
   }
+  constexpr bool UPD = (ABL & BLK_UPD) != 0;
+  static_assert(!UPD || (DOTS && BP::LATT), "fused vector update: lattice blocks, fused dot products");
+  auto update_interior = [&](uint32_t g) {
+    const uint32_t *lrow = bp.lattice + (uint64_t)g * BLOCK_LATTICE_WORDS;
+    const uint32_t hdr = lrow[54], lo = lrow[27 + 13];
+    const uint32_t len = ((hdr & 255u) * P - 1u) * (((hdr >> 8) & 255u) * P - 1u) * (((hdr >> 16) & 255u) * P - 1u);
+    const uint32_t hi = lo + len < bp.upd_end ? lo + len : bp.upd_end;
+    if (bp.upd_mode == 2u) block_update_run<2>(bp, lo, hi, t);
+    else block_update_run<1>(bp, lo, hi, t);
+  };
   const uint32_t ba0 = bp.wg_block[w], ba1 = bp.wg_block[w + 1];
   const uint32_t bb0 = bp.n_parts > 1 ? bp.wg_block[bp.n_wg + 1 + w] : 0u, bb1 = bp.n_parts > 1 ? bp.wg_block[bp.n_wg + 1 + w + 1] : 0u;
   const uint32_t nba = ba1 - ba0, b1 = nba + (bb1 - bb0);
@@ -2267,7 +2285,7 @@
       enter_block(rt0, n_runs, m);
       __syncthreads();
     }
-    BP::decode_and_gather(a, A, rt0, staged, use_lattice ? lat_tab + (b & 1u) * BLOCK_LATTICE_WORDS : nullptr, a_, b_);
+    if constexpr (!UPD) BP::decode_and_gather(a, A, rt0, staged, use_lattice ? lat_tab + (b & 1u) * BLOCK_LATTICE_WORDS : nullptr, a_, b_);
   } else
     BP::issue_gather(a, A);
 
@@ -2287,6 +2305,7 @@
         nx_r1 = bp.run_off[p1 + 1];
       }
       if constexpr (use_lattice) { if (t < BLOCK_LATTICE_WORDS) lat_word = bp.lattice[(uint64_t)p1 * BLOCK_LATTICE_WORDS + t]; }
+      if constexpr (UPD) update_interior(p1);
     }
     if (gp + 1 == boundary) {
       if constexpr (BP::PACK) {
@@ -2403,6 +2422,7 @@
           rt[BLOCK_MAX_RUNS + t] = run_dof;
         }
       }
+      if constexpr (UPD) vmem_drain();
       __syncthreads();
       BP5_PRIO_WO_HI
       if constexpr (CARRY) {
@@ -2506,6 +2526,14 @@
   };
 
   while (gp < gp_end) {
+    if constexpr (UPD) {
+      if (gp == 0) {
+        update_interior(pb);
+        vmem_drain();
+        __syncthreads();
+        BP::decode_and_gather(a, A, run_tab, staged, lat_tab, a_, b_);
+      }
+    }
     prefetch_list();
     BP5_PRIO_HI BP::issue_loads(a, bp, B, abm, lane_ok, gp + 1 < gp_end); BP5_PRIO_LO
     const uint32_t entA2 = entry(gp + 2);
@@ -3351,7 +3379,7 @@
 
 enum { SC_GH = 0, SC_DH, SC_GG, SC_GDG, SC_ALPHA, SC_BETA, SC_ALPHA_OLD, SC_BETA_OLD, SC_RES, SC_RES0, SC_TOL, SC_R0 ,
        SC_COUNT = SC_R0 + 7 };
-enum { ST_DONE = 0, ST_ITER, ST_PENDING, ST_MAXIT, ST_BREAKDOWN, ST_COUNT };
+enum { ST_DONE = 0, ST_ITER, ST_PENDING, ST_MAXIT, ST_BREAKDOWN, ST_HOLD, ST_COUNT };
 
 static __global__ void copy_constrained_components_kernel(const uint32_t *cdofs, uint32_t n, const double *src, double *dst, size_t ld)
 {
@@ -3506,12 +3534,10 @@
     p = fma(beta, p, -(di * rn));
   }
 }
-template <int MODE, int U = 2, bool ZV = false, bool NTX = false>
-__global__ void __launch_bounds__(VB) cgm_update_kernel(double *p, double *r, typename std::conditional<ZV, double, const double>::type *v, double *x,
-                                                       const double *diag, size_t n, const double *sc, const int *st)
-{
-  const bool done = st[ST_DONE];
-  if (done && !st[ST_PENDING]) return;
+template <int MODE, int U, bool ZV, bool NTX>
+__device__ __forceinline__ void cgm_update_body(double *p, double *r, typename std::conditional<ZV, double, const double>::type *v, double *x,
+                                                const double *diag, size_t n, const double *sc, const int *st, const bool done)
+{
   const double alpha = sc[SC_ALPHA], beta = sc[SC_BETA];
   const double aob = (MODE == 2 || done) ? sc[SC_ALPHA_OLD] / sc[SC_BETA_OLD] : 0.0;
   const bool epi_odd = done && (st[ST_ITER] & 1);
@@ -3566,6 +3592,70 @@
     }
   }
 }
+template <int MODE, int U = 2, bool ZV = false, bool NTX = false>
+__global__ void __launch_bounds__(VB) cgm_update_kernel(double *p, double *r, typename std::conditional<ZV, double, const double>::type *v, double *x,
+                                                       const double *diag, size_t n, const double *sc, const int *st)
+{
+  const bool done = st[ST_DONE];
+  if (done && !st[ST_PENDING]) return;
+  cgm_update_body<MODE, U, ZV, NTX>(p, r, v, x, diag, n, sc, st, done);
+}
+template <int MODE, int U, bool NTX>
+__global__ void __launch_bounds__(VB) cgm_update_rest_kernel(double *p, double *r, const double *v, double *x, const double *diag, size_t first, size_t n,
+                                                            const double *sc, const int *st)
+{
+  if (st[ST_DONE]) return;
+  cgm_update_body<MODE, U, false, NTX>(p + first, r + first, v + first, x + first, diag ? diag + first : nullptr, n, sc, st, false);
+}
+#ifndef BP5_UPD_UNROLL
+#define BP5_UPD_UNROLL 3
+#endif
+template <int MODE>
+__device__ __forceinline__ void block_update_run(const BlockPlan &bp, uint32_t lo, uint32_t hi, int t)
+{
+  static_assert(MODE == 1 || MODE == 2, "the first iteration's p comes from cgm_init_kernel");
+  constexpr int U = BP5_UPD_UNROLL;
+  constexpr uint32_t TRIP = 2u * 256u;
+  const double *sc = bp.upd_sc;
+  const double alpha = sc[SC_ALPHA], beta = sc[SC_BETA];
+  const double aob = MODE == 2 ? sc[SC_ALPHA_OLD] / sc[SC_BETA_OLD] : 0.0;
+  double *const p = bp.upd_p, *const r = bp.upd_r, *const x = bp.upd_x;
+  const double *const v = bp.upd_v, *const diag = bp.upd_diag;
+  for (uint32_t base = lo + 2u * (uint32_t)t; base < hi; base += TRIP * U) {
+    bp5_d2u pv[U], rv[U], vv[U], xv[U];
+#pragma unroll
+    for (int u = 0; u < U; ++u) {
+      const uint32_t i = base + (uint32_t)u * TRIP;
+      pv[u] = rv[u] = vv[u] = xv[u] = bp5_d2u{0.0, 0.0};
+      if (i + 1 < hi) {
+        pv[u] = __builtin_nontemporal_load(reinterpret_cast<const bp5_d2u *>(p + i));
+        rv[u] = __builtin_nontemporal_load(reinterpret_cast<const bp5_d2u *>(r + i));
+        vv[u] = __builtin_nontemporal_load(reinterpret_cast<const bp5_d2u *>(v + i));
+        if (MODE == 2) xv[u] = __builtin_nontemporal_load(reinterpret_cast<const bp5_d2u *>(x + i));
+      } else if (i < hi) {
+        pv[u].x = __builtin_nontemporal_load(p + i); rv[u].x = __builtin_nontemporal_load(r + i); vv[u].x = __builtin_nontemporal_load(v + i);
+        if (MODE == 2) xv[u].x = __builtin_nontemporal_load(x + i);
+      }
+    }
+#pragma unroll
+    for (int u = 0; u < U; ++u) {
+      const uint32_t i = base + (uint32_t)u * TRIP;
+      if (i >= hi) continue;
+      const bool pair = i + 1 < hi;
+      double p0 = pv[u].x, p1 = pv[u].y, r0 = rv[u].x, r1 = rv[u].y, x0 = xv[u].x, x1 = xv[u].y;
+      cgm_update_one<MODE>(p0, r0, vv[u].x, x0, diag ? diag[i] : 1.0, false, false, alpha, beta, aob);
+      if (pair) {
+        cgm_update_one<MODE>(p1, r1, vv[u].y, x1, diag ? diag[i + 1] : 1.0, false, false, alpha, beta, aob);
+        *reinterpret_cast<bp5_d2u *>(p + i) = bp5_d2u{p0, p1};
+        *reinterpret_cast<bp5_d2u *>(r + i) = bp5_d2u{r0, r1};
+        if (MODE == 2) __builtin_nontemporal_store(bp5_d2u{x0, x1}, reinterpret_cast<bp5_d2u *>(x + i));
+      } else {
+        p[i] = p0; r[i] = r0;
+        if (MODE == 2) __builtin_nontemporal_store(x0, x + i);
+      }
+    }
+  }
+}
 template <int MODE>
 __global__ void __launch_bounds__(256) cgm_pack_updated_kernel(const uint32_t *idx, uint32_t n, const double *p, const double *r, const double *v,
                                                              const double *diag, const double *sc, const int *st, double *buf)
@@ -3615,7 +3705,7 @@
 static __global__ void cgm_control_kernel(double *sc, int *st);
 __device__ __forceinline__ void cgm_control_step(double *sc, int *st)
 {
-  if (st[ST_DONE]) { st[ST_PENDING] = 0; return; }
+  if (st[ST_DONE]) { if (!st[ST_HOLD]) st[ST_PENDING] = 0; return; }
   const double *R = sc + SC_R0;
   if (!(R[0] == R[0]) || R[0] == 0.0) { st[ST_BREAKDOWN] = 1; st[ST_DONE] = 1; return; }
   sc[SC_ALPHA_OLD] = sc[SC_ALPHA];
@@ -3682,11 +3772,11 @@
   acc[1] = acc[0];
   block_reduce_store<2>(acc, partials);
 }
-static __global__ void cgm_init_control_kernel(double *sc, int *st)
+static __global__ void cgm_init_control_kernel(double *sc, int *st, int hold)
 {
   sc[SC_RES0] = sc[SC_RES] = sqrt(sc[SC_GG]);
   sc[SC_ALPHA] = sc[SC_BETA] = sc[SC_ALPHA_OLD] = sc[SC_BETA_OLD] = 0.0;
-  st[ST_ITER] = 0; st[ST_PENDING] = 0; st[ST_BREAKDOWN] = 0;
+  st[ST_ITER] = 0; st[ST_PENDING] = 0; st[ST_BREAKDOWN] = 0; st[ST_HOLD] = hold;
   st[ST_DONE] = (sc[SC_RES] <= sc[SC_TOL]) ? 1 : 0;
 }
 
diff --git a/deal-and-ceed-on-gpu_amd/matrix_free.py b/deal-and-ceed-on-gpu_amd/matrix_free.py
--- a/deal-and-ceed-on-gpu_amd/matrix_free.py
+++ b/deal-and-ceed-on-gpu_amd/matrix_free.py
@@ -148,7 +148,7 @@
         _lib.check(_lib.lib().bp5_mf_set_streaming(self.handle, int(policy)))
 
     TUNE = {"lattice_indices": 0, "early_gather": 1, "combine_signal": 2, "boundary_first": 3, "fold_small": 4, "update_unroll": 5,
-            "update_flat": 6, "update_nt": 7, "combine_wg_per_cu": 8, "interior_stores": 9, "ghost_combine_on_comm": 10, "face_carry": 11}
+            "update_flat": 6, "update_nt": 7, "combine_wg_per_cu": 8, "interior_stores": 9, "ghost_combine_on_comm": 10, "face_carry": 11, "fused_update": 12}
 
     def set_tuning(self, knob, value):
         _lib.check(_lib.lib().bp5_mf_set_tuning(self.handle, int(self.TUNE.get(knob, knob)), int(value)))
diff --git a/include/bp5.h b/include/bp5.h
--- a/include/bp5.h
+++ b/include/bp5.h
@@ -150,7 +150,8 @@
 int bp5_mf_set_streaming(bp5_mf *mf, int policy);
 enum { BP5_TUNE_LATTICE_INDICES = 0, BP5_TUNE_EARLY_GATHER = 1, BP5_TUNE_COMBINE_SIGNAL = 2, BP5_TUNE_BOUNDARY_FIRST = 3,
        BP5_TUNE_FOLD_SMALL = 4, BP5_TUNE_UPDATE_UNROLL = 5, BP5_TUNE_UPDATE_FLAT = 6, BP5_TUNE_UPDATE_NT = 7, BP5_TUNE_COMBINE_WG_PER_CU = 8,
-       BP5_TUNE_INTERIOR_STORES = 9, BP5_TUNE_GHOST_COMBINE_ON_COMM = 10, BP5_TUNE_FACE_CARRY = 11, BP5_TUNE_COUNT = 12 };
+       BP5_TUNE_INTERIOR_STORES = 9, BP5_TUNE_GHOST_COMBINE_ON_COMM = 10, BP5_TUNE_FACE_CARRY = 11, BP5_TUNE_FUSED_UPDATE = 12,
+       BP5_TUNE_COUNT = 13 };
 int bp5_mf_set_tuning(bp5_mf *mf, int knob, int value);
 int bp5_mf_get_tuning(const bp5_mf *mf, int knob, int *value);
 int bp5_mf_wait_value_available(bp5_mf *mf, int *available);
```
